# ak110/object_detector

Measured on AMD Instinct MI355X. Metric: images_per_sec, higher is better.
Workload: dtype f16

## Files before the change

object_detector_amd/csrc/conv_8ph.hip:

```cpp
#include "conv_8ph_tile.h"
#include "conv_common.h"

namespace {

struct E8Entry {
  int BM;
  bool (*variant)(int ksize, bool pw, int epi, int epi2, const void** fn, const char** name);
};
const E8Entry g_e8[] = {{256, od_conv_8ph_variant_mf4}, {224, od_conv_8ph_variant_mf3}, {192, od_conv_8ph_variant_mf2},
                        {160, od_conv_8ph_variant_mf1}};
constexpr int kNumE8 = sizeof(g_e8) / sizeof(g_e8[0]);

}

int od_conv_8ph_num_cfgs() { return kNumE8; }

long od_conv_8ph_tiles(int idx, int M, int Cout) { return (long)od_ceil_div(M, g_e8[idx].BM) * od_ceil_div(Cout, E_BN); }
double od_conv_8ph_tile_cost(int idx, int nk) { return 13.0 + 1.78 * nk * (0.5 + 0.0625 * (g_e8[idx].BM / 32)); }

bool od_conv_8ph_can_fuse_pointwise(const ConvKP& p) { return p.splitk == 1 && p.Cout == E_BN && p.Cout2 == 128; }

bool od_conv_8ph_select(int idx, const ConvKP& p, int ksize, ConvKernelInfo* info) {
  if (idx < 0 || idx >= kNumE8) return false;
  if ((p.Cin & 63) != 0 || p.tconv) return false;
  if (p.x_bytes >= 0x7F000000u || p.w_bytes >= 0x7F000000u || p.x_bytes == 0) return false;
  const E8Entry& e = g_e8[idx];
  const bool pw = p.w2 != nullptr;
  if (p.nseg > 1 && (ksize != 3 || pw || p.stride != 1 || p.res_mode != OD_RES_NONE)) return false;
  const size_t epi = (size_t)(e.BM / 2) * (E_BN + 4) * 4;
  const int epi1 = od_epi_of(p);
  const int epi2 = (pw && epi1 != OD_EPI_RT) ? od_epi(p.act2, OD_RES_NONE, false) : OD_EPI_RT;
  const void* fn;
  const char* name;
  if (!e.variant(ksize, pw, epi1, epi2, &fn, &name) &&
      !e.variant(ksize, pw, OD_EPI_RT, OD_EPI_RT, &fn, &name))
    return false;
  *info = {fn, name, e.BM, E_BN, E_BK, 512, epi > (size_t)2 * E_BUF ? epi : (size_t)2 * E_BUF};
  return true;
}
```

object_detector_amd/csrc/conv_8ph_inst.hip:

```cpp
#include "conv_8ph_kernel.h"

#ifndef OD_E8_MF1
#error "compile with -DOD_E8_MF1=1..4"
#endif

namespace {

struct E8Variant {
  int ksize;
  bool pw;
  int epi, epi2;
  const void* fn;
  const char* name;
};
#define OD_E8V(KS, PW, SEG, EPI, EPI2)                                                                                  \
  {KS, PW, EPI, EPI2, (const void*)&od_conv_8ph<KS, OD_E8_MF1, EPI, EPI2, PW, SEG>,                                     \
   "od_conv_8ph<" #KS ", " OD_STR(OD_E8_MF1) ", " OD_STR(EPI) ", " OD_STR(EPI2) ", " #PW ", " #SEG ">"}
const E8Variant g_variants[] = {
    OD_E8V(1, false, false, OD_EPI_RT, OD_EPI_RT),
    OD_E8V(1, false, false, OD_EPI_LEAKY_NONE_F16, OD_EPI_RT),
    OD_E8V(1, false, false, OD_EPI_ELU_NONE_F16, OD_EPI_RT),
    OD_E8V(1, false, false, OD_EPI_ELU_UP2_F16, OD_EPI_RT),
    OD_E8V(1, false, false, OD_EPI_ELU_NONE_F32, OD_EPI_RT),
    OD_E8V(3, false, true, OD_EPI_RT, OD_EPI_RT),
    OD_E8V(3, false, true, OD_EPI_LEAKY_NONE_F16, OD_EPI_RT),
    OD_E8V(3, false, true, OD_EPI_LEAKY_SAME_F16, OD_EPI_RT),
    OD_E8V(3, false, true, OD_EPI_ELU_NONE_F16, OD_EPI_RT),
    OD_E8V(3, false, true, OD_EPI_ELU_UP2_F16, OD_EPI_RT),
    OD_E8V(3, false, true, OD_EPI_LINEAR_NONE_F32, OD_EPI_RT),
    OD_E8V(3, false, true, OD_EPI_LEAKY_NONE_F32, OD_EPI_RT),
    OD_E8V(3, false, true, OD_EPI_ELU_NONE_F32, OD_EPI_RT),
    OD_E8V(1, true, false, OD_EPI_RT, OD_EPI_RT),
    OD_E8V(3, true, false, OD_EPI_RT, OD_EPI_RT),
    OD_E8V(3, true, false, OD_EPI_LEAKY_NONE_F16, OD_EPI_LEAKY_NONE_F16),
    OD_E8V(3, true, false, OD_EPI_LEAKY_SAME_F16, OD_EPI_LEAKY_NONE_F16),
};

}

#define OD_CAT_(a, b) a##b
#define OD_CAT(a, b) OD_CAT_(a, b)
bool OD_CAT(od_conv_8ph_variant_mf, OD_E8_MF1)(int ksize, bool pw, int epi, int epi2, const void** fn, const char** name) {
  for (const E8Variant& v : g_variants)
    if (v.ksize == ksize && v.pw == pw && v.epi == epi && v.epi2 == epi2) {
      *fn = v.fn;
      *name = v.name;
      return true;
    }
  return false;
}
```

object_detector_amd/csrc/conv_8ph_kernel.h:

```cpp
#pragma once
#include "conv_8ph_tile.h"
#include "conv_common.h"

namespace {

constexpr int E_ALO = 0, E_AHI = E_REGION, E_BLO = 2 * E_REGION, E_BHI = 3 * E_REGION;

struct TapWalk {
  int c0, tap, tapoff, dx;
  int sel_tap;
};

constexpr unsigned E_OOB = 0x80000000u;

template <int MT, int NF = 4, bool KEEP = false>
static __device__ __forceinline__ void e8_epilogue_rt(const ConvKP& p, f32x4 (&acc)[MT][NF], int m0w, int n0w, int l15,
                                                          int lq, f16x8 (*keep)[NF / 2] = nullptr, int mrows = MT * 16,
                                                          const float* pre_sc = nullptr, const float* pre_bi = nullptr) {
  unsigned pb[MT], ppix[MT];
#pragma unroll
  for (int i = 0; i < MT; ++i) {
    const int m = m0w + i * 16 + l15;
    pb[i] = (unsigned)m / (unsigned)p.HoWo;
    ppix[i] = (unsigned)m - pb[i] * (unsigned)p.HoWo;
  }
#pragma unroll
  for (int pr = 0; pr < NF / 2; ++pr) {
    const int n = n0w + (2 * pr + (lq & 1)) * 16 + (lq >> 1) * 8;
    const bool nok = n < p.Cout;
    float sc[8], bi[8];
    if (pre_sc) {
#pragma unroll
      for (int e = 0; e < 8; ++e) {
        sc[e] = pre_sc[e];
        bi[e] = pre_bi[e];
      }
    } else {
      const f32x4 s0 = *(const f32x4*)(p.scale + n), s1 = *(const f32x4*)(p.scale + n + 4);
      const f32x4 b0 = *(const f32x4*)(p.bias + n), b1 = *(const f32x4*)(p.bias + n + 4);
#pragma unroll
      for (int e = 0; e < 4; ++e) {
        sc[e] = s0[e];
        sc[4 + e] = s1[e];
        bi[e] = b0[e];
        bi[4 + e] = b1[e];
      }
    }
    f16x8 rv[MT];
#pragma unroll
    for (int i = 0; i < MT; ++i) {
      const int m = m0w + i * 16 + l15;
      f16x8 r = {0, 0, 0, 0, 0, 0, 0, 0};
      if (nok && m < p.M && p.res_mode != OD_RES_NONE) {
        long long roff;
        if (p.res_mode == OD_RES_SAME) {
          roff = (long long)m * p.Cout + n;
        } else {
          const unsigned ho = ppix[i] / (unsigned)p.Wo, wo = ppix[i] - ho * (unsigned)p.Wo;
          roff = ((long long)(pb[i] * (unsigned)(p.Ho >> 1) + (ho >> 1)) * (p.Wo >> 1) + (wo >> 1)) * p.Cout + n;
        }
        r = *(const f16x8*)(p.res + roff);
      }
      rv[i] = r;
    }
#pragma unroll
    for (int i = 0; i < MT; ++i) {
      const int m = m0w + i * 16 + l15;
      const bool ok = nok && m < p.M && i * 16 + l15 < mrows;
      float v[8];
#pragma unroll
      for (int e = 0; e < 4; ++e) {
        float a = acc[i][2 * pr][e], bq = acc[i][2 * pr + 1][e];
        od_permlane16_swap(a, bq);
        v[e] = a;
        v[4 + e] = bq;
      }
#pragma unroll
      for (int e = 0; e < 8; ++e) v[e] = v[e] * sc[e] + bi[e];
      if (p.act == OD_ACT_LEAKY) {
#pragma unroll
        for (int e = 0; e < 8; ++e) v[e] = od_leaky(v[e], p.alpha);
      } else if (p.act == OD_ACT_ELU) {
#pragma unroll
        for (int e = 0; e < 8; ++e) v[e] = v[e] > 0.f ? v[e] : p.alpha * od_expm1_fast(v[e]);
      }
      if (p.res_mode != OD_RES_NONE) {
#pragma unroll
        for (int e = 0; e < 8; ++e) v[e] += (float)rv[i][e];
      }
      if (ok) {
        const long long ooff = (long long)pb[i] * p.obs + (long long)ppix[i] * p.ops + n;
        if (p.out_f32) {
          float* o = (float*)p.out + ooff;
          *(f32x4*)o = f32x4{v[0], v[1], v[2], v[3]};
          *(f32x4*)(o + 4) = f32x4{v[4], v[5], v[6], v[7]};
        } else {
          f16x8 h;
#pragma unroll
          for (int e = 0; e < 8; ++e) h[e] = (f16)v[e];
          *(f16x8*)((f16*)p.out + ooff) = h;
        }
      }
      if (KEEP) {
        f16x8 h;
#pragma unroll
        for (int e = 0; e < 8; ++e) h[e] = (f16)v[e];
        keep[i][pr] = h;
      }
    }
  }
}

template <int EPI, int MT, int NF, bool KEEP>
static __device__ __forceinline__ void e8_epilogue_fixed(const ConvKP& p, f32x4 (&acc)[MT][NF], int m0w, int n0w, int l15, int lq,
                                                         f16x8 (*keep)[NF / 2], int mrows, const float* pre_sc,
                                                         const float* pre_bi) {
  constexpr int ACT = od_epi_act(EPI), RES = od_epi_res(EPI);
  constexpr bool F32 = od_epi_f32(EPI);
  unsigned orow[MT], rrow[RES != OD_RES_NONE ? MT : 1];
#pragma unroll
  for (int i = 0; i < MT; ++i) {
    const unsigned m = (unsigned)min(m0w + i * 16 + l15, p.M - 1);
    const unsigned b = m / (unsigned)p.HoWo, pix = m - b * (unsigned)p.HoWo;
    orow[i] = b * (unsigned)p.obs + pix * (unsigned)p.ops;
    if (RES == OD_RES_SAME) rrow[i] = m * (unsigned)p.Cout;
    if (RES == OD_RES_UP2) {
      const unsigned ho = pix / (unsigned)p.Wo, wo = pix - ho * (unsigned)p.Wo;
      rrow[i] = ((b * (unsigned)(p.Ho >> 1) + (ho >> 1)) * (unsigned)(p.Wo >> 1) + (wo >> 1)) * (unsigned)p.Cout;
    }
  }
#pragma unroll
  for (int pr = 0; pr < NF / 2; ++pr) {
    const int n = n0w + (2 * pr + (lq & 1)) * 16 + (lq >> 1) * 8;
    const bool nok = n < p.Cout;
    float sc[8], bi[8];
    if (pre_sc) {
#pragma unroll
      for (int e = 0; e < 8; ++e) {
        sc[e] = pre_sc[e];
        bi[e] = pre_bi[e];
      }
    } else {
      const f32x4 s0 = *(const f32x4*)(p.scale + n), s1 = *(const f32x4*)(p.scale + n + 4);
      const f32x4 b0 = *(const f32x4*)(p.bias + n), b1 = *(const f32x4*)(p.bias + n + 4);
#pragma unroll
      for (int e = 0; e < 4; ++e) {
        sc[e] = s0[e];
        sc[4 + e] = s1[e];
        bi[e] = b0[e];
        bi[4 + e] = b1[e];
      }
    }
    f16x8 rv[RES != OD_RES_NONE ? MT : 1];
    if (RES != OD_RES_NONE) {
      const unsigned nr = nok ? (unsigned)n : 0u;
#pragma unroll
      for (int i = 0; i < MT; ++i) rv[i] = *(const f16x8*)(p.res + (rrow[i] + nr));
    }
#pragma unroll
    for (int i = 0; i < MT; ++i) {
      f32x4 a = acc[i][2 * pr], bq = acc[i][2 * pr + 1];
      od_permlane16_swap4(a, bq);
      float v[8] = {a[0], a[1], a[2], a[3], bq[0], bq[1], bq[2], bq[3]};
#pragma unroll
      for (int e = 0; e < 8; ++e) v[e] = v[e] * sc[e] + bi[e];
      if (ACT == OD_ACT_LEAKY) {
#pragma unroll
        for (int e = 0; e < 8; ++e) v[e] = od_leaky(v[e], p.alpha);
      } else if (ACT == OD_ACT_ELU) {
#pragma unroll
        for (int e = 0; e < 8; ++e) v[e] = od_elu_select(v[e], p.alpha);
      }
      if (RES != OD_RES_NONE) {
#pragma unroll
        for (int e = 0; e < 8; ++e) v[e] += (float)rv[i][e];
      }
      f16x8 h;
      if (!F32 || KEEP) {
#pragma unroll
        for (int e = 0; e < 8; ++e) h[e] = (f16)v[e];
      }
      if (nok && m0w + i * 16 + l15 < p.M && i * 16 + l15 < mrows) {
        const unsigned ooff = orow[i] + (unsigned)n;
        if (F32) {
          float* o = (float*)p.out + ooff;
          *(f32x4*)o = f32x4{v[0], v[1], v[2], v[3]};
          *(f32x4*)(o + 4) = f32x4{v[4], v[5], v[6], v[7]};
        } else {
          *(f16x8*)((f16*)p.out + ooff) = h;
        }
      }
      if (KEEP) keep[i][pr] = h;
    }
  }
}

template <int MT, int NF = 4, bool KEEP = false, int EPI = OD_EPI_RT>
static __device__ __forceinline__ void e8_epilogue_direct(const ConvKP& p, f32x4 (&acc)[MT][NF], int m0w, int n0w, int l15,
                                                          int lq, f16x8 (*keep)[NF / 2] = nullptr, int mrows = MT * 16,
                                                          const float* pre_sc = nullptr, const float* pre_bi = nullptr) {
  if constexpr (EPI == OD_EPI_RT)
    e8_epilogue_rt<MT, NF, KEEP>(p, acc, m0w, n0w, l15, lq, keep, mrows, pre_sc, pre_bi);
  else
    e8_epilogue_fixed<EPI, MT, NF, KEEP>(p, acc, m0w, n0w, l15, lq, keep, mrows, pre_sc, pre_bi);
}

template <int KS, int MF1, int EPI, int EPI2, bool PW, bool SEG>
__global__ __launch_bounds__(512, 2) void od_conv_8ph(ConvKP p_in) {
  constexpr int MF0 = 4, MT = MF0 + MF1, WROWS = MT * 16, BM = 2 * WROWS;
  extern __shared__ __attribute__((aligned(16))) char smem[];
  const int tid = threadIdx.x;
  const int lane = tid & 63;
  const int wave = __builtin_amdgcn_readfirstlane(tid >> 6);
  const int wr = wave >> 2, wc = wave & 3;
  const int l15 = lane & 15, lq = lane >> 4;

  int logical;
  {
    const int nt = p_in.mtiles * p_in.ntiles;
    const int pid = p_in.splitk > 1 ? (int)blockIdx.x / p_in.splitk : (int)blockIdx.x;
    const int q = nt >> 3, r = nt & 7, xcd = pid & 7, loc = pid >> 3;
    logical = (xcd < r ? xcd * (q + 1) : r * (q + 1) + (xcd - r) * q) + loc;
  }
  int tm = logical / p_in.ntiles;
  const int tn = logical - tm * p_in.ntiles;
  ConvKP p_seg;
  if (SEG) p_seg = p_in;
  if (SEG && p_in.nseg > 1) {
    int sg = 0;
    if (tm >= p_in.seg_tile0[1]) sg = 1;
    if (p_in.nseg > 2 && tm >= p_in.seg_tile0[2]) sg = 2;
    tm -= p_in.seg_tile0[sg];
    p_seg.x = p_in.seg_x[sg];
    p_seg.out = p_in.seg_out[sg];
    p_seg.H = p_seg.Ho = p_in.seg_H[sg];
    p_seg.W = p_seg.Wo = p_in.seg_W[sg];
    p_seg.HoWo = p_seg.H * p_seg.W;
    p_seg.M = p_in.seg_M[sg];
    p_seg.x_bytes = (unsigned)p_seg.M * (unsigned)p_in.Cin * 2u;
    if (p_in.obs == 0) p_seg.obs = (long long)p_seg.HoWo * p_in.Cout;
  }
  const ConvKP& p = SEG ? p_seg : p_in;
  const int m0 = tm * BM, n0 = tn * E_BN;
  const int nk_all = p.Ktot / E_BK;
  const int ks0 = p.splitk > 1 ? ((int)blockIdx.x % p.splitk) * p.steps_per_split : 0;
  const int nk = p.splitk > 1 ? min(p.steps_per_split, nk_all - ks0) : nk_all;
  if (nk <= 0) return;

  const int rr = tid >> 3;
  const int lc = (tid & 7) ^ (rr & 7);
  int a_base[2][2];
  unsigned a_vmask[2][2];
  unsigned a_sel[2][2];
#pragma unroll
  for (int s = 0; s < 2; ++s)
#pragma unroll
    for (int j = 0; j < 2; ++j) {
      const int m = m0 + j * WROWS + s * 64 + rr;
      a_vmask[s][j] = 0u;
      a_base[s][j] = 0;
      if (m < p.M && (s == 0 || rr < MF1 * 16)) {
        const unsigned b = (unsigned)m / (unsigned)p.HoWo;
        const unsigned pix = (unsigned)m - b * (unsigned)p.HoWo;
        const unsigned ho = pix / (unsigned)p.Wo;
        const unsigned wo = pix - ho * (unsigned)p.Wo;
        const int hi0 = (int)ho * p.stride - p.pad, wi0 = (int)wo * p.stride - p.pad;
        a_base[s][j] = ((((int)b * p.H + hi0 + p.pad) * p.W + wi0 + p.pad) * p.Cin + lc * 8) * 2;
#pragma unroll
        for (int t = 0; t < KS * KS; ++t) {
          const int hi = hi0 + t / KS, wi = wi0 + t % KS;
          if ((unsigned)hi < (unsigned)p.H && (unsigned)wi < (unsigned)p.W) a_vmask[s][j] |= 1u << t;
        }
      }
    }
  int w_off[2][2];
#pragma unroll
  for (int s = 0; s < 2; ++s)
#pragma unroll
    for (int j = 0; j < 2; ++j) {
      const int n = n0 + (2 * j + (rr >> 5)) * 64 + s * 32 + (rr & 31);
      w_off[s][j] = (n * p.Kstride + lc * 8 + ks0 * E_BK) * 2;
    }
  const __amdgpu_buffer_rsrc_t rs_x = __builtin_amdgcn_make_buffer_rsrc(
      (void*)(p.x - (long long)p.pad * (p.W + 1) * p.Cin), 0, (int)(p.x_bytes + (unsigned)(p.pad * (p.W + 1) * p.Cin * 2)),
      0x00020000);
  const __amdgpu_buffer_rsrc_t rs_w = __builtin_amdgcn_make_buffer_rsrc((void*)p.w, 0, (int)p.w_bytes, 0x00020000);
  auto blds16 = [&](const __amdgpu_buffer_rsrc_t& rs, unsigned voff, int soff, char* lptr) {
    __builtin_amdgcn_raw_ptr_buffer_load_lds(rs, (__attribute__((address_space(3))) void*)lptr, 16, (int)voff, soff, 0, 0);
  };

  auto walk_init = [&](TapWalk& w, int kt) {
    const int k0 = kt * E_BK;
    if (KS == 3) {
      w.sel_tap = -1;
      w.tap = k0 / p.Cin;
      w.c0 = k0 - w.tap * p.Cin;
      const int dy = w.tap / 3;
      w.dx = w.tap - dy * 3;
      w.tapoff = (dy * p.W + w.dx) * p.Cin;
    } else {
      w.sel_tap = -1;
      w.tap = 0;
      w.c0 = k0;
      w.dx = 0;
      w.tapoff = 0;
    }
  };
  auto walk_next = [&](TapWalk& w) {
    w.c0 += E_BK;
    if (KS == 3 && w.c0 >= p.Cin) {
      w.c0 = 0;
      ++w.tap;
      if (++w.dx == 3) {
        w.dx = 0;
        w.tapoff += (p.W - 2) * p.Cin;
      } else {
        w.tapoff += p.Cin;
      }
    }
  };
  TapWalk walk_lo, walk_hi;
  walk_init(walk_lo, ks0);
  walk_init(walk_hi, ks0);

  char* const piece = smem + wave * 1024;
  auto stage_a = [&](int s, TapWalk& w, int buf) {
    const int koff = w.tapoff + w.c0;
    char* dst = piece + buf * E_BUF + (s ? E_AHI : E_ALO);
    if (w.sel_tap != w.tap) {
      w.sel_tap = w.tap;
#pragma unroll
      for (int j = 0; j < 2; ++j) a_sel[s][j] = ((a_vmask[s][j] >> w.tap) & 1u) ? (unsigned)a_base[s][j] : E_OOB;
    }
#pragma unroll
    for (int j = 0; j < 2; ++j) blds16(rs_x, a_sel[s][j], koff * 2, dst + j * 8192);
    walk_next(w);
  };
  auto stage_b = [&](int s, int t, int buf) {
    char* dst = piece + buf * E_BUF + (s ? E_BHI : E_BLO);
#pragma unroll
    for (int j = 0; j < 2; ++j) blds16(rs_w, (unsigned)w_off[s][j], t * (E_BK * 2), dst + j * 8192);
  };

  const int w2buf = ((nk - 1) & 1) ^ 1;
  const __amdgpu_buffer_rsrc_t rs_w2 =
      __builtin_amdgcn_make_buffer_rsrc((void*)(PW ? p.w2 : p.w), 0, (int)(PW ? p.w2_bytes : p.w_bytes), 0x00020000);
  auto stage_w2 = [&](int ks) {
#pragma unroll
    for (int h = 0; h < 2; ++h)
      blds16(rs_w2, (unsigned)(((h * 64 + rr) * p.K2stride + lc * 8) * 2), ks * (E_BK * 2),
             piece + w2buf * E_BUF + ks * E_REGION + h * 8192);
  };

  f32x4 acc[MT][4];
#pragma unroll
  for (int i = 0; i < MT; ++i)
#pragma unroll
    for (int j = 0; j < 4; ++j) acc[i][j] = f32x4{0.f, 0.f, 0.f, 0.f};

  stage_a(0, walk_lo, 0);
  stage_b(0, 0, 0);
  stage_b(1, 0, 0);
  stage_a(1, walk_hi, 0);
  if (nk > 1) {
    stage_a(0, walk_lo, 1);
    stage_b(0, 1, 1);
    wait_vmcnt<8>();
  } else {
    wait_vmcnt<0>();
  }
  __builtin_amdgcn_s_barrier();

  const int fa = (wr * 64 + l15) * 128 + ((lq ^ (l15 & 7)) * 16);
  const int fb = (wc * 32 + l15) * 128 + ((lq ^ (l15 & 7)) * 16);

  f16x8 xa[MF0][2], wlo[2][2], whi[2][2];
  auto ldf = [&](f16x8& dst, const char* src) { dst = *(const f16x8*)src; };
  auto mma = [&](f32x4& c, const f16x8& a, const f16x8& b) {
    c = __builtin_amdgcn_mfma_f32_16x16x32_f16(a, b, c, 0, 0, 0);
  };

  auto L0 = [&](int t) {
    const char* cur = smem + (t & 1) * E_BUF;
#pragma unroll
    for (int f = 0; f < 2; ++f)
#pragma unroll
      for (int kh = 0; kh < 2; ++kh) ldf(wlo[f][kh], cur + E_BLO + ((fb + f * 2048) ^ (kh * 64)));
#pragma unroll
    for (int f = 0; f < MF0; ++f)
#pragma unroll
      for (int kh = 0; kh < 2; ++kh) ldf(xa[f][kh], cur + E_ALO + ((fa + f * 2048) ^ (kh * 64)));
    if (t + 1 < nk) {
      stage_b(1, t + 1, (t & 1) ^ 1);
      wait_vmcnt<8>();
    } else if (PW) {
      stage_w2(0);
      wait_vmcnt<2>();
    } else {
      wait_vmcnt<0>();
    }
  };
  auto L1 = [&](int t) {
    const char* cur = smem + (t & 1) * E_BUF;
#pragma unroll
    for (int f = 0; f < 2; ++f)
#pragma unroll
      for (int kh = 0; kh < 2; ++kh) ldf(whi[f][kh], cur + E_BHI + ((fb + f * 2048) ^ (kh * 64)));
    if (t + 1 < nk) {
      stage_a(1, walk_hi, (t & 1) ^ 1);
      wait_vmcnt<8>();
    } else if (PW) {
      stage_w2(1);
    } else {
      wait_vmcnt<0>();
    }
  };
  auto L2 = [&](int t) {
    const char* cur = smem + (t & 1) * E_BUF;
#pragma unroll
    for (int f = 0; f < MF1; ++f)
#pragma unroll
      for (int kh = 0; kh < 2; ++kh) ldf(xa[f][kh], cur + E_AHI + ((fa + f * 2048) ^ (kh * 64)));
    if (t + 2 < nk) stage_a(0, walk_lo, t & 1);
    if (PW && t + 1 == nk) stage_w2(2);
  };
  auto L3 = [&](int t) {
    if (t + 2 < nk) {
      stage_b(0, t + 2, t & 1);
      wait_vmcnt<8>();
    } else if (PW && t + 1 == nk) {
      stage_w2(3);
    } else {
      wait_vmcnt<0>();
    }
  };
  auto M = [&](int ph) {
    __builtin_amdgcn_s_setprio(1);
#pragma unroll
    for (int kh = 0; kh < 2; ++kh)
#pragma unroll
      for (int i = 0; i < ((ph < 2) ? MF0 : MF1); ++i)
#pragma unroll
        for (int j = 0; j < 2; ++j) {
          if (ph == 0) mma(acc[i][j], wlo[j][kh], xa[i][kh]);
          if (ph == 1) mma(acc[i][2 + j], whi[j][kh], xa[i][kh]);
          if (ph == 2) mma(acc[MF0 + i][2 + j], whi[j][kh], xa[i][kh]);
          if (ph == 3) mma(acc[MF0 + i][j], wlo[j][kh], xa[i][kh]);
        }
    __builtin_amdgcn_s_setprio(0);
  };

  if (wr == 0) {
    for (int t = 0; t < nk; ++t) {
      L0(t);
      M(0);
      __builtin_amdgcn_s_barrier();
      L1(t);
      M(1);
      __builtin_amdgcn_s_barrier();
      L2(t);
      M(2);
      __builtin_amdgcn_s_barrier();
      L3(t);
      M(3);
      __builtin_amdgcn_s_barrier();
    }
  } else {
    L0(0);
    __builtin_amdgcn_s_barrier();
    for (int t = 0; t < nk; ++t) {
      M(0);
      L1(t);
      __builtin_amdgcn_s_barrier();
      M(1);
      L2(t);
      __builtin_amdgcn_s_barrier();
      M(2);
      L3(t);
      __builtin_amdgcn_s_barrier();
      M(3);
      if (t + 1 < nk) {
        L0(t + 1);
        __builtin_amdgcn_s_barrier();
      }
    }
  }
  __syncthreads();

  if constexpr (PW) {
    const int rg = wave >> 2, cg = wave & 3;
    float sc2[8], bi2[8];
    {
      const int n2 = cg * 32 + (lq & 1) * 16 + (lq >> 1) * 8;
      const f32x4 s0 = *(const f32x4*)(p.scale2 + n2), s1 = *(const f32x4*)(p.scale2 + n2 + 4);
      const f32x4 b0 = *(const f32x4*)(p.bias2 + n2), b1 = *(const f32x4*)(p.bias2 + n2 + 4);
#pragma unroll
      for (int e = 0; e < 4; ++e) {
        sc2[e] = s0[e];
        sc2[4 + e] = s1[e];
        bi2[e] = b0[e];
        bi2[4 + e] = b1[e];
      }
    }
    f16x8 ykeep[MT][2];
    od_mfma_results_ready();
    e8_epilogue_direct<MT, 4, true, EPI>(p, acc, m0 + wr * WROWS, n0 + wc * 64, l15, lq, ykeep);
    ConvKP p2 = p;
    p2.scale = p.scale2;
    p2.bias = p.bias2;
    p2.act = p.act2;
    p2.alpha = p.alpha2;
    p2.res_mode = OD_RES_NONE;
    p2.out = (void*)p.out2;
    p2.out_f32 = 0;
    p2.Cout = p.Cout2;
    p2.obs = (long long)p.HoWo * p.Cout2;
    p2.ops = p.Cout2;
    char* const ybuf = smem + (w2buf ^ 1) * E_BUF;
    const char* const wbuf = smem + w2buf * E_BUF;
    const int fy = (rg * 64 + l15) * 128 + ((lq ^ (l15 & 7)) * 16);
    const int fw = (cg * 32 + l15) * 128 + ((lq ^ (l15 & 7)) * 16);
#pragma unroll
    for (int half = 0; half < 2; ++half) {
      if (wr == half) {
#pragma unroll
        for (int i = 0; i < MT; ++i)
#pragma unroll
          for (int pr = 0; pr < 2; ++pr) {
            const int row = i * 16 + l15;
            const int chunk = (2 * pr + (lq & 1)) * 2 + (lq >> 1);
            *(f16x8*)(ybuf + wc * E_REGION + row * 128 + ((chunk ^ (row & 7)) * 16)) = ykeep[i][pr];
          }
      }
      asm volatile("s_waitcnt lgkmcnt(0)" ::: "memory");
      __builtin_amdgcn_s_barrier();
      f32x4 acc2[4][2];
#pragma unroll
      for (int i = 0; i < 4; ++i)
#pragma unroll
        for (int f = 0; f < 2; ++f) acc2[i][f] = f32x4{0.f, 0.f, 0.f, 0.f};
#pragma unroll
      for (int ks = 0; ks < 4; ++ks)
#pragma unroll
        for (int kh = 0; kh < 2; ++kh) {
          f16x8 wf[2], yf[4];
#pragma unroll
          for (int f = 0; f < 2; ++f) wf[f] = *(const f16x8*)(wbuf + ks * E_REGION + ((fw + f * 2048) ^ (kh * 64)));
#pragma unroll
          for (int i = 0; i < 4; ++i) yf[i] = *(const f16x8*)(ybuf + ks * E_REGION + ((fy + i * 2048) ^ (kh * 64)));
#pragma unroll
          for (int i = 0; i < 4; ++i)
#pragma unroll
            for (int f = 0; f < 2; ++f) acc2[i][f] = __builtin_amdgcn_mfma_f32_16x16x32_f16(wf[f], yf[i], acc2[i][f], 0, 0, 0);
        }
      od_mfma_results_ready();
      e8_epilogue_direct<4, 2, false, EPI2>(p2, acc2, m0 + half * WROWS + rg * 64, cg * 32, l15, lq, nullptr, WROWS - rg * 64, sc2, bi2);
      if (half == 0) {
        asm volatile("s_waitcnt lgkmcnt(0)" ::: "memory");
        __builtin_amdgcn_s_barrier();
      }
    }
  } else if (EPI == OD_EPI_RT && p.splitk > 1) {
    conv_epilogue<E_BN, 2, 4, MT, 4, 512>(p, smem, acc, m0, n0, tid, wr, wc, l15, lq);
  } else {
    od_mfma_results_ready();
    e8_epilogue_direct<MT, 4, false, EPI>(p, acc, m0 + wr * WROWS, n0 + wc * 64, l15, lq);
  }
}

}
```

object_detector_amd/csrc/conv_common.h:

```cpp
#pragma once
#include "common.h"

struct ConvKP {
  const f16* x;
  const f16* w;
  const float* scale;
  const float* bias;
  const f16* res;
  void* out;
  const f16* zero;
  int H, W, Cin, Ho, Wo, Cout;
  int stride, pad;
  int Kstride, Ktot, M, HoWo;
  int act;
  float alpha;
  int res_mode, out_f32;
  long long obs, ops;
  int mtiles, ntiles;
  int splitk, steps_per_split;
  float* ws;
  int Mq;
  int tconv, Hs, Ws;
  unsigned x_bytes, w_bytes;
  float* stats;
  const f16* w2;
  const float* scale2;
  const float* bias2;
  f16* out2;
  int Cout2, act2;
  float alpha2;
  unsigned w2_bytes;
  int K2stride;
  int nseg;
  int seg_tile0[4];
  const f16* seg_x[3];
  void* seg_out[3];
  int seg_H[3], seg_W[3], seg_M[3];
  int off32;
};

static __device__ __forceinline__ void glds16(const void* gptr, void* lptr) {
  __builtin_amdgcn_global_load_lds((const __attribute__((address_space(1))) void*)gptr,
                                   (__attribute__((address_space(3))) void*)lptr, 16, 0, 0);
}

static __device__ __forceinline__ float od_expm1_fast(float v) {
  const float poly = v * (1.f + v * (0.5f + v * (1.f / 6 + v * (1.f / 24 + v * (1.f / 120 + v * (1.f / 720))))));
  return v > -0.25f ? poly : __expf(v) - 1.f;
}

static __device__ __forceinline__ float od_elu_select(float v, float alpha) {
  const float poly = v * (1.f + v * (0.5f + v * (1.f / 6 + v * (1.f / 24 + v * (1.f / 120 + v * (1.f / 720))))));
  const float ex = __expf(v) - 1.f;
  const float em = v > -0.25f ? poly : ex;
  const float neg = alpha * em;
  return v > 0.f ? v : neg;
}

#define OD_EPI_RT -1
#define OD_EPI_LEAKY_NONE_F16 1
#define OD_EPI_LEAKY_SAME_F16 5
#define OD_EPI_ELU_NONE_F16 2
#define OD_EPI_ELU_UP2_F16 10
#define OD_EPI_LINEAR_NONE_F32 16
#define OD_EPI_LEAKY_NONE_F32 17
#define OD_EPI_ELU_NONE_F32 18
constexpr int od_epi(int act, int res_mode, bool out_f32) { return act | (res_mode << 2) | ((int)out_f32 << 4); }
static_assert(od_epi(OD_ACT_LEAKY, OD_RES_NONE, false) == OD_EPI_LEAKY_NONE_F16 &&
                  od_epi(OD_ACT_LEAKY, OD_RES_SAME, false) == OD_EPI_LEAKY_SAME_F16 &&
                  od_epi(OD_ACT_ELU, OD_RES_NONE, false) == OD_EPI_ELU_NONE_F16 &&
                  od_epi(OD_ACT_ELU, OD_RES_UP2, false) == OD_EPI_ELU_UP2_F16 &&
                  od_epi(OD_ACT_LINEAR, OD_RES_NONE, true) == OD_EPI_LINEAR_NONE_F32 &&
                  od_epi(OD_ACT_LEAKY, OD_RES_NONE, true) == OD_EPI_LEAKY_NONE_F32 &&
                  od_epi(OD_ACT_ELU, OD_RES_NONE, true) == OD_EPI_ELU_NONE_F32,
              "OD_EPI_* literals");
constexpr int od_epi_act(int epi) { return epi & 3; }
constexpr int od_epi_res(int epi) { return (epi >> 2) & 3; }
constexpr bool od_epi_f32(int epi) { return ((epi >> 4) & 1) != 0; }
static inline int od_epi_of(const ConvKP& p) {
  return (p.off32 && p.splitk <= 1 && !p.tconv && !p.stats) ? od_epi(p.act, p.res_mode, p.out_f32 != 0) : OD_EPI_RT;
}
#define OD_STR_(x) #x
#define OD_STR(x) OD_STR_(x)

static __device__ __forceinline__ void od_permlane16_swap(float& a, float& b) {
  asm volatile("s_nop 1\n\tv_permlane16_swap_b32 %0, %1\n\ts_nop 1" : "+v"(a), "+v"(b));
}
static __device__ __forceinline__ void od_permlane16_swap4(f32x4& a, f32x4& b) {
  float a0 = a[0], a1 = a[1], a2 = a[2], a3 = a[3], b0 = b[0], b1 = b[1], b2 = b[2], b3 = b[3];
  asm volatile(
      "s_nop 1\n\tv_permlane16_swap_b32 %0, %4\n\tv_permlane16_swap_b32 %1, %5\n\tv_permlane16_swap_b32 %2, %6\n\t"
      "v_permlane16_swap_b32 %3, %7\n\ts_nop 1"
      : "+v"(a0), "+v"(a1), "+v"(a2), "+v"(a3), "+v"(b0), "+v"(b1), "+v"(b2), "+v"(b3));
  a = f32x4{a0, a1, a2, a3};
  b = f32x4{b0, b1, b2, b3};
}
static __device__ __forceinline__ void od_mfma_results_ready() {
  __builtin_amdgcn_sched_barrier(0);
  asm volatile("s_nop 15\n\ts_nop 15" ::: "memory");
  __builtin_amdgcn_sched_barrier(0);
}

static __device__ __forceinline__ float od_leaky(float v, float alpha) { return fmaxf(v, v * alpha); }

template <int N>
static __device__ __forceinline__ void wait_vmcnt() {
  asm volatile("s_waitcnt vmcnt(%0)" ::"n"(N) : "memory");
}


static __device__ __forceinline__ int od_tconv_pixel(const ConvKP& p, unsigned m, unsigned BM) {
  const unsigned t = m / BM, r = m - t * BM;
  const unsigned cls = t & 3u, idx = (t >> 2) * BM + r;
  if (idx >= (unsigned)p.Mq) return -1;
  const unsigned HsWs = (unsigned)(p.Hs * p.Ws);
  const unsigned b = idx / HsWs, q = idx - b * HsWs;
  const unsigned i = q / (unsigned)p.Ws, j = q - i * (unsigned)p.Ws;
  return (int)(b * (unsigned)p.HoWo + (2u * i + (cls >> 1)) * (unsigned)p.Wo + 2u * j + (cls & 1u));
}

template <int BN, int WM, int WN, int MT, int NTL, int NT = WM * WN * 64, bool STATS = false, int EPI = OD_EPI_RT>
static __device__ __forceinline__ void conv_epilogue(const ConvKP& p, char* smem, f32x4 (&acc)[MT][NTL], int m0, int n0,
                                                     int tid, int wm, int wn, int l15, int lq) {
  constexpr int WTM = MT * 16, WTN = NTL * 16, SLD = BN + 4;
  constexpr bool FX = EPI != OD_EPI_RT;
  static_assert(!(FX && STATS), "the statistics epilogue has no policy");
  const int act = FX ? od_epi_act(EPI) : p.act, res_mode = FX ? od_epi_res(EPI) : p.res_mode;
  const bool out_f32 = FX ? od_epi_f32(EPI) : p.out_f32 != 0;
  const bool splitk = !FX && p.splitk > 1, tconv = !FX && p.tconv;
  float* stg = (float*)smem;
  constexpr int CH = BN / 8;
  constexpr int RPP = NT / CH;
  const int c8 = (tid % CH) * 8;
  const int n = n0 + c8;
  float sc[8], bi[8];
  if (!STATS) {
    const f32x4 s0 = *(const f32x4*)(p.scale + n), s1 = *(const f32x4*)(p.scale + n + 4);
    const f32x4 b0 = *(const f32x4*)(p.bias + n), b1 = *(const f32x4*)(p.bias + n + 4);
#pragma unroll
    for (int e = 0; e < 4; ++e) {
      sc[e] = s0[e];
      sc[4 + e] = s1[e];
      bi[e] = b0[e];
      bi[4 + e] = b1[e];
    }
  }
  float st0[STATS ? 8 : 1], st1[STATS ? 8 : 1];
  if (STATS) {
#pragma unroll
    for (int e = 0; e < 8; ++e) st0[e] = st1[e] = 0.f;
  }
  constexpr int NPASS = (WTM + RPP - 1) / RPP;
  constexpr bool RAGGED = (WTM % RPP) != 0;
  f16x8 resv[WM][NPASS];
  if (res_mode != OD_RES_NONE && !splitk) {
#pragma unroll
    for (int wr = 0; wr < WM; ++wr)
#pragma unroll
      for (int ps = 0; ps < NPASS; ++ps) {
        int m = m0 + wr * WTM + ps * RPP + tid / CH;
        f16x8 r = {0, 0, 0, 0, 0, 0, 0, 0};
        if (RAGGED && ps * RPP + tid / CH >= WTM) m = p.M;
        if (tconv && m < p.M) m = od_tconv_pixel(p, (unsigned)m, WM * MT * 16);
        if (m >= 0 && m < p.M && n < p.Cout) {
          long long roff;
          if (res_mode == OD_RES_SAME) {
            roff = (long long)m * p.Cout + n;
          } else {
            const unsigned b = (unsigned)m / (unsigned)p.HoWo;
            const unsigned pix = (unsigned)m - b * (unsigned)p.HoWo;
            const unsigned ho = pix / (unsigned)p.Wo, wo = pix - ho * (unsigned)p.Wo;
            roff = ((long long)(b * (unsigned)(p.Ho >> 1) + (ho >> 1)) * (p.Wo >> 1) + (wo >> 1)) * p.Cout + n;
          }
          r = *(const f16x8*)(p.res + roff);
        }
        resv[wr][ps] = r;
      }
  }
#pragma unroll
  for (int wr = 0; wr < WM; ++wr) {
    if (wm == wr) {
#pragma unroll
      for (int j = 0; j < NTL; ++j) {
        const int nl = wn * WTN + j * 16 + lq * 4;
#pragma unroll
        for (int i = 0; i < MT; ++i) *(f32x4*)(stg + (i * 16 + l15) * SLD + nl) = acc[i][j];
      }
    }
    __syncthreads();
    if (splitk) {
      float* slab = p.ws + (long long)((int)blockIdx.x % p.splitk) * p.M * p.Cout;
#pragma unroll
      for (int ps = 0; ps < NPASS; ++ps) {
        const int row = ps * RPP + tid / CH;
        const int m = (RAGGED && row >= WTM) ? p.M : m0 + wr * WTM + row;
        if (m < p.M && n < p.Cout) {
          float* o = slab + (long long)m * p.Cout + n;
          *(f32x4*)o = *(const f32x4*)(stg + row * SLD + c8);
          *(f32x4*)(o + 4) = *(const f32x4*)(stg + row * SLD + c8 + 4);
        }
      }
      if (wr + 1 < WM) __syncthreads();
      continue;
    }
#pragma unroll
    for (int ps = 0; ps < NPASS; ++ps) {
      const int row = ps * RPP + tid / CH;
      int m = (RAGGED && row >= WTM) ? p.M : m0 + wr * WTM + row;
      if (tconv && m < p.M) m = od_tconv_pixel(p, (unsigned)m, WM * MT * 16);
      if (m >= 0 && m < p.M && n < p.Cout) {
        const f32x4 v0 = *(const f32x4*)(stg + row * SLD + c8);
        const f32x4 v1 = *(const f32x4*)(stg + row * SLD + c8 + 4);
        float v[8] = {v0[0], v0[1], v0[2], v0[3], v1[0], v1[1], v1[2], v1[3]};
        if (!STATS) {
#pragma unroll
          for (int e = 0; e < 8; ++e) v[e] = v[e] * sc[e] + bi[e];
        }
        if (STATS) {
        } else if (act == OD_ACT_LEAKY) {
#pragma unroll
          for (int e = 0; e < 8; ++e) v[e] = od_leaky(v[e], p.alpha);
        } else if (act == OD_ACT_ELU) {
#pragma unroll
          for (int e = 0; e < 8; ++e) v[e] = FX ? od_elu_select(v[e], p.alpha) : (v[e] > 0.f ? v[e] : p.alpha * od_expm1_fast(v[e]));
        }
        if (!STATS && res_mode != OD_RES_NONE) {
#pragma unroll
          for (int e = 0; e < 8; ++e) v[e] += (float)resv[wr][ps][e];
        }
        const unsigned b = (unsigned)m / (unsigned)p.HoWo;
        const unsigned pix = (unsigned)m - b * (unsigned)p.HoWo;
        const long long ooff = FX ? (long long)(b * (unsigned)p.obs + pix * (unsigned)p.ops + (unsigned)n)
                                  : (long long)b * p.obs + (long long)pix * p.ops + n;
        if (out_f32) {
          float* o = (float*)p.out + ooff;
          *(f32x4*)o = f32x4{v[0], v[1], v[2], v[3]};
          *(f32x4*)(o + 4) = f32x4{v[4], v[5], v[6], v[7]};
        } else {
          f16x8 h;
#pragma unroll
          for (int e = 0; e < 8; ++e) h[e] = (f16)v[e];
          *(f16x8*)((f16*)p.out + ooff) = h;
          if (STATS) {
#pragma unroll
            for (int e = 0; e < 8; ++e) {
              const float q = (float)h[e];
              st0[e] += q;
              st1[e] += q * q;
            }
          }
        }
      }
    }
    if (wr + 1 < WM) __syncthreads();
  }
  if (STATS) {
    static_assert(CH == 8 || CH == 16 || CH == 32, "BN must be 64, 128 or 256");
#pragma unroll
    for (int off = CH; off < 64; off <<= 1) {
#pragma unroll
      for (int e = 0; e < 8; ++e) {
        st0[e] += __shfl_xor(st0[e], off, 64);
        st1[e] += __shfl_xor(st1[e], off, 64);
      }
    }
    __syncthreads();
    float* red = (float*)smem;
    const int wv = tid >> 6, ln = tid & 63;
    if (ln < CH) {
#pragma unroll
      for (int e = 0; e < 8; ++e) {
        red[(wv * CH + ln) * 16 + e] = st0[e];
        red[(wv * CH + ln) * 16 + 8 + e] = st1[e];
      }
    }
    __syncthreads();
    if (tid < CH && n < p.Cout) {
      float a[8], b[8];
#pragma unroll
      for (int e = 0; e < 8; ++e) a[e] = b[e] = 0.f;
      for (int w2 = 0; w2 < NT / 64; ++w2) {
#pragma unroll
        for (int e = 0; e < 8; ++e) {
          a[e] += red[(w2 * CH + tid) * 16 + e];
          b[e] += red[(w2 * CH + tid) * 16 + 8 + e];
        }
      }
      float* row = p.stats + (long long)(m0 / (WM * WTM)) * 2 * p.Cout;
#pragma unroll
      for (int e = 0; e < 8; ++e) {
        row[n + e] = a[e];
        row[p.Cout + n + e] = b[e];
      }
    }
  }
}

struct ConvKernelInfo {
  const void* fn;
  const char* name;
  int BM, BN, BK, threads;
  size_t lds;
};

int od_conv_igemm_num_cfgs();
bool od_conv_igemm_select(int cfg, int ksize, int Cin, bool want_stats, int epi, ConvKernelInfo* info);
int od_conv_finish_prepare(const ConvKP& p, od_launches* L);
int od_conv_8ph_num_cfgs();
long od_conv_8ph_tiles(int idx, int M, int Cout);
double od_conv_8ph_tile_cost(int idx, int nk);
bool od_conv_8ph_can_fuse_pointwise(const ConvKP& p);
bool od_conv_8ph_select(int idx, const ConvKP& p, int ksize, ConvKernelInfo* info);
bool od_conv_8ph_variant_mf4(int ksize, bool pw, int epi, int epi2, const void** fn, const char** name);
bool od_conv_8ph_variant_mf3(int ksize, bool pw, int epi, int epi2, const void** fn, const char** name);
bool od_conv_8ph_variant_mf2(int ksize, bool pw, int epi, int epi2, const void** fn, const char** name);
bool od_conv_8ph_variant_mf1(int ksize, bool pw, int epi, int epi2, const void** fn, const char** name);
bool od_tconv_small_supported(const od_conv_desc* d);
int od_tconv_small_prepare(od_ctx* ctx, const od_conv_desc* d, od_launches* L);
bool od_conv_rdirect_supported(const od_conv_desc* d);
int od_conv_rdirect_prepare(od_ctx* ctx, const od_conv_desc* d, od_launches* L);
bool od_conv_stream3_supported(const od_conv_desc* d);
int od_conv_stream3_prepare(od_ctx* ctx, const od_conv_desc* d, od_launches* L);
```

object_detector_amd/csrc/conv_dispatch.hip:

```cpp
#include <string.h>

#include "conv_common.h"

namespace {

int pick_cfg(const od_ctx* ctx, int M, int Cin, int Cout, int ksize, bool e8_ok, bool throughput) {
  const int cus = ctx->num_cu;
  const int cfg_e8 = od_conv_igemm_num_cfgs();
  const bool spec_ok = (Cin % 64) == 0;
  if (Cout <= 64) return (ksize == 3 && od_ceil_div(M, 128) >= 8 * cus) ? 1 : 3;
  const long t128 = (long)od_ceil_div(M, 128) * od_ceil_div(Cout, 128);
  if (ksize == 1) {
    if (!spec_ok) return 3;
    if (M <= 4096) return (M >= 2048 && Cin >= 512) ? 6 : 3;
    if (M <= 16384) return 7;
    if (Cout < 256) return 3;
    if (t128 < cus) return 4;
  }
  if (!spec_ok) return t128 >= 2L * cus ? 0 : 2;
  const int nk = od_ceil_div(ksize * ksize * Cin, 64);
  if (throughput && e8_ok && ksize == 3 && Cout >= 192 && M >= 2048) {
    double best = t128 >= cus ? t128 * (7.5 + 1.07 * nk) * 0.5 : t128 * (10.0 + 0.55 * nk);
    int pick = t128 >= cus ? 4 : (Cout <= 256 ? 7 : 5);
    for (int i = 0; i < od_conv_8ph_num_cfgs(); ++i) {
      const long tiles = od_conv_8ph_tiles(i, M, Cout);
      if (tiles * 3 < cus) continue;
      const double c = (double)tiles * od_conv_8ph_tile_cost(i, nk);
      if (c < 0.95 * best) {
        best = c / 0.95;
        pick = cfg_e8 + i;
      }
    }
    return pick;
  }
  if (t128 >= cus) {
    if (Cout == 128) return 2;
    const double c13 = (double)od_ceil_div((int)t128, 2 * cus) * (7.5 + 1.07 * nk);
    double best = 0.93 * c13;
    int pick = 4;
    for (int i = 0; e8_ok && i < od_conv_8ph_num_cfgs(); ++i) {
      const double c = (double)((od_conv_8ph_tiles(i, M, Cout) + cus - 1) / cus) * od_conv_8ph_tile_cost(i, nk);
      if (c < best) {
        best = c;
        pick = cfg_e8 + i;
      }
    }
    return pick;
  }
  if (Cout <= 256) return M < 2048 ? 3 : 7;
  return (M >= 2048 && 2 * t128 <= cus) ? 7 : 5;
}

int conv_describe(const od_ctx* ctx, const od_conv_desc* d, bool want_stats, od_conv_desc* v, ConvKP* kp) {
  if (d && d->nseg > 1) {
    OD_REQUIRE(d->nseg <= 3, "od_conv2d_fwd: nseg %d > 3", d->nseg);
    OD_REQUIRE(d->ksize == 3 && d->stride == 1 && d->res_mode == OD_RES_NONE && !d->w2 && !want_stats && !d->transposed,
               "od_conv2d_fwd: a grouped launch (nseg > 1) is a 3x3 stride-1 layer without residual / w2 / bn_partials / "
               "transposed mode");
    for (int i = 0; i < d->nseg; ++i)
      OD_REQUIRE(d->seg_x[i] && d->seg_out[i] && d->seg_H[i] > 0 && d->seg_W[i] > 0, "od_conv2d_fwd: segment %d is incomplete", i);
  }
  OD_REQUIRE(ctx && d, "od_conv2d_fwd: null ctx/desc");
  *v = *d;
  const bool grouped = d->nseg > 1;
  if (grouped) {
    v->x = d->seg_x[0];
    v->out = d->seg_out[0];
    v->H = d->seg_H[0];
    v->W = d->seg_W[0];
  }
  d = v;
  OD_REQUIRE(d->x && d->w && d->scale && d->bias && d->out, "od_conv2d_fwd: null tensor");
  OD_REQUIRE(d->ksize == 1 || d->ksize == 3, "od_conv2d_fwd: ksize %d unsupported", d->ksize);
  OD_REQUIRE(d->stride == 1 || d->stride == 2, "od_conv2d_fwd: stride %d unsupported", d->stride);
  OD_REQUIRE(d->B > 0 && d->H > 0 && d->W > 0 && d->Cin > 0 && d->Cout > 0, "od_conv2d_fwd: bad dims");
  OD_REQUIRE(d->Cin % 8 == 0 && d->Cout % 8 == 0, "od_conv2d_fwd: Cin/Cout must be multiples of 8 (got %d/%d)",
             d->Cin, d->Cout);
  OD_REQUIRE(d->res_mode == OD_RES_NONE || d->res, "od_conv2d_fwd: res_mode set but res is null");
  OD_REQUIRE(d->act >= OD_ACT_LINEAR && d->act <= OD_ACT_ELU, "od_conv2d_fwd: bad act");
  OD_REQUIRE(d->act != OD_ACT_LEAKY || (d->alpha >= 0.f && d->alpha <= 1.f), "od_conv2d_fwd: leaky slope must be in [0, 1]");
  ConvKP& p = *kp;
  p.pad = d->ksize / 2;
  p.tconv = d->transposed != 0;
  if (p.tconv)
    OD_REQUIRE(d->ksize == 3 && d->stride == 2 && d->Cin % 64 == 0,
               "od_conv2d_fwd: transposed mode is the backward-data of a 3x3 stride-2 conv (Cin %% 64 == 0)");
  p.H = p.tconv ? 2 * d->H : d->H;
  p.W = p.tconv ? 2 * d->W : d->W;
  p.stride = p.tconv ? 1 : d->stride;
  p.Hs = d->H;
  p.Ws = d->W;
  p.Ho = (p.H + 2 * p.pad - d->ksize) / p.stride + 1;
  p.Wo = (p.W + 2 * p.pad - d->ksize) / p.stride + 1;
  if (d->res_mode == OD_RES_UP2)
    OD_REQUIRE(p.Ho % 2 == 0 && p.Wo % 2 == 0, "od_conv2d_fwd: OD_RES_UP2 needs even output size");
  const long long M64 = (long long)d->B * p.Ho * p.Wo;
  OD_REQUIRE(M64 * d->Cout < (1LL << 31) && (long long)d->B * d->H * d->W * d->Cin < (1LL << 31),
             "od_conv2d_fwd: tensor too large for 32-bit element offsets");
  p.HoWo = p.Ho * p.Wo;
  long long Mg = 0;
  long long seg_x_max = 0;
  for (int i = 0; grouped && i < d->nseg; ++i) {
    const long long Mi = (long long)d->B * d->seg_H[i] * d->seg_W[i];
    Mg += Mi;
    seg_x_max = seg_x_max > Mi * d->Cin ? seg_x_max : Mi * d->Cin;
  }
  OD_REQUIRE(!grouped || (Mg * d->Cout < (1LL << 31) && seg_x_max < (1LL << 31)),
             "od_conv2d_fwd: grouped launch too large for 32-bit element offsets");
  p.M = grouped ? (int)Mg : (int)M64;
  p.nseg = grouped ? d->nseg : 0;

  if (want_stats)
    OD_REQUIRE(!p.tconv && d->out_dtype == OD_DT_F16 && d->act == OD_ACT_LINEAR && d->res_mode == OD_RES_NONE,
               "od_conv2d_fwd: bn_partials needs the raw convolution (f16 output, no activation, no residual, no transposed "
               "gather; scale / bias are NOT applied)");
  if (d->w2) {
    OD_REQUIRE(d->scale2 && d->bias2 && d->out2 && d->Cout2 > 0 && d->Cout2 % 8 == 0,
               "od_conv2d_fwd: w2 needs scale2, bias2, out2 and Cout2 (a multiple of 8)");
    OD_REQUIRE(d->act2 >= OD_ACT_LINEAR && d->act2 <= OD_ACT_ELU, "od_conv2d_fwd: bad act2");
    OD_REQUIRE(d->act2 != OD_ACT_LEAKY || (d->alpha2 >= 0.f && d->alpha2 <= 1.f), "od_conv2d_fwd: leaky slope (alpha2) must be in [0, 1]");
    OD_REQUIRE(d->out_dtype == OD_DT_F16 && !p.tconv && !want_stats && d->Cout % 8 == 0 &&
                   (d->out_batch_stride == 0 || d->out_batch_stride == (long long)p.HoWo * d->Cout) &&
                   (d->out_pix_stride == 0 || d->out_pix_stride == d->Cout),
               "od_conv2d_fwd: w2 (the consuming pointwise layer) needs a dense f16 output of the first layer");
  }
  p.x = (const f16*)d->x;
  p.w = (const f16*)d->w;
  p.scale = d->scale;
  p.bias = d->bias;
  p.res = (const f16*)d->res;
  p.out = d->out;
  p.zero = (const f16*)ctx->zero_page;
  p.Cin = d->Cin;
  p.Cout = d->Cout;
  p.Ktot = d->ksize * d->ksize * d->Cin;
  p.Kstride = od_round_up(p.Ktot, 64);
  p.act = d->act;
  p.alpha = d->alpha;
  p.res_mode = d->res_mode;
  p.out_f32 = d->out_dtype == OD_DT_F32;
  p.stats = d->bn_partials;
  p.w2 = nullptr;
  p.scale2 = d->scale2;
  p.bias2 = d->bias2;
  p.out2 = (f16*)d->out2;
  p.Cout2 = d->Cout2;
  p.act2 = d->act2;
  p.alpha2 = d->alpha2;
  p.K2stride = od_round_up(d->Cout, 64);
  p.w2_bytes = (unsigned)((long long)od_round_up(d->Cout2 > 0 ? d->Cout2 : 1, 256) * p.K2stride * 2);
  p.x_bytes = (unsigned)((grouped ? seg_x_max : (long long)d->B * d->H * d->W * d->Cin) * 2);
  p.w_bytes = (unsigned)((long long)od_round_up(d->Cout, 256) * p.Kstride * 2);
  p.obs = d->out_batch_stride ? d->out_batch_stride : (long long)p.HoWo * d->Cout;
  p.ops = d->out_pix_stride ? d->out_pix_stride : d->Cout;
  long long hw_max = p.HoWo;
  for (int i = 0; grouped && i < d->nseg; ++i) hw_max = hw_max > (long long)d->seg_H[i] * d->seg_W[i] ? hw_max : (long long)d->seg_H[i] * d->seg_W[i];
  p.off32 = p.obs >= 0 && p.ops >= 0 && (long long)d->B * p.obs < (1LL << 31) &&
            (long long)(d->B - 1) * p.obs + (hw_max - 1) * p.ops + d->Cout < (1LL << 31);
  p.splitk = 1;
  p.steps_per_split = 0;
  p.ws = (float*)d->splitk_workspace;
  return OD_OK;
}

int conv_choose_cfg(const od_ctx* ctx, const od_conv_desc* d, const ConvKP& p, bool want_stats, int* cfg_out) {
  int cfg = d->tile_cfg;
  if (cfg < 0)
    cfg = pick_cfg(ctx, p.M, d->Cin, d->Cout, d->ksize, !want_stats && !p.tconv && (long long)p.x_bytes < 0x7F000000LL, cfg == -2);
  const int cfg_e8 = od_conv_igemm_num_cfgs();
  OD_REQUIRE(cfg < cfg_e8 + od_conv_8ph_num_cfgs(), "od_conv2d_fwd: tile_cfg %d out of range", cfg);
  OD_REQUIRE(!(want_stats && cfg >= cfg_e8), "od_conv2d_fwd: bn_partials is supported by the table kernels only (tile_cfg %d)", cfg);
  OD_REQUIRE(!p.tconv || cfg < cfg_e8, "od_conv2d_fwd: transposed mode runs on the table kernels only (tile_cfg %d)", cfg);
  *cfg_out = cfg;
  return OD_OK;
}

int conv_select(int cfg, const od_conv_desc* d, const ConvKP& p, bool want_stats, ConvKernelInfo* k) {
  const int cfg_e8 = od_conv_igemm_num_cfgs();
  if (cfg >= cfg_e8) {
    if (od_conv_8ph_select(cfg - cfg_e8, p, d->ksize, k)) return OD_OK;
    od_set_error("od_conv2d_fwd: tile_cfg %d (8-phase kernel) needs Cin %% 64 == 0 and no transposed gather", cfg);
    return OD_ERR_INVALID;
  }
  if (od_conv_igemm_select(cfg, d->ksize, d->Cin, want_stats, od_epi_of(p), k)) return OD_OK;
  od_set_error("od_conv2d_fwd: tile_cfg %d needs Cin %% %d == 0 for 3x3 (Cin = %d); use cfg 0-3", cfg, k->BK, d->Cin);
  return OD_ERR_INVALID;
}

void conv_tile_kp(const od_conv_desc* d, const ConvKernelInfo& k, ConvKP* kp) {
  ConvKP& p = *kp;
  p.mtiles = od_ceil_div(p.M, k.BM);
  if (p.nseg > 1) {
    int t0 = 0;
    for (int i = 0; i < 3; ++i) {
      const bool used = i < d->nseg;
      p.seg_tile0[i] = t0;
      p.seg_x[i] = used ? (const f16*)d->seg_x[i] : nullptr;
      p.seg_out[i] = used ? d->seg_out[i] : nullptr;
      p.seg_H[i] = used ? d->seg_H[i] : 0;
      p.seg_W[i] = used ? d->seg_W[i] : 0;
      p.seg_M[i] = d->B * p.seg_H[i] * p.seg_W[i];
      t0 += od_ceil_div(p.seg_M[i], k.BM);
    }
    p.seg_tile0[3] = t0;
    p.mtiles = t0;
    if (!d->out_batch_stride) p.obs = 0;
  }
  p.Mq = 0;
  if (p.tconv) {
    p.Mq = p.M / 4;
    p.mtiles = 4 * od_ceil_div(p.Mq, k.BM);
    p.M = p.mtiles * k.BM;
  }
  p.ntiles = od_ceil_div(d->Cout, k.BN);
}

int conv_prepare(od_ctx* ctx, const od_conv_desc* desc, bool want_stats, od_launches* L) {
  od_conv_desc v;
  ConvKP p;
  if (int rc = conv_describe(ctx, desc, want_stats, &v, &p)) return rc;
  const od_conv_desc* d = &v;
  const bool grouped = p.nseg > 1;
  if (d->tile_cfg < 0 && !want_stats && !grouped) {
    if (p.tconv && od_tconv_small_supported(d)) return od_tconv_small_prepare(ctx, d, L);
    if (od_conv_rdirect_supported(d)) return od_conv_rdirect_prepare(ctx, d, L);
    if (!p.tconv && od_conv_stream3_supported(d)) return od_conv_stream3_prepare(ctx, d, L);
  }
  int cfg;
  if (int rc = conv_choose_cfg(ctx, d, p, want_stats, &cfg)) return rc;
  const bool use_e8 = cfg >= od_conv_igemm_num_cfgs();
  if (grouped && !(use_e8 && d->Cin % 64 == 0)) {
    od_conv_desc q = *d;
    q.nseg = 0;
    for (int i = 0; i < d->nseg; ++i) {
      q.x = d->seg_x[i];
      q.out = d->seg_out[i];
      q.H = d->seg_H[i];
      q.W = d->seg_W[i];
      if (int rc = conv_prepare(ctx, &q, false, L)) return rc;
    }
    return OD_OK;
  }
  ConvKernelInfo k;
  if (int rc = conv_select(cfg, d, p, want_stats, &k)) return rc;
  conv_tile_kp(d, k, &p);
  if (d->bn_partials) {
    const long long need = (long long)p.mtiles * 2 * d->Cout * 4;
    if (d->bn_partials_bytes < need) {
      od_set_error("od_conv2d_fwd: bn_partials holds %lld bytes, %d rows x 2 x %d channels need %lld", (long long)d->bn_partials_bytes,
                   p.mtiles, d->Cout, need);
      return OD_ERR_WORKSPACE;
    }
  }
  if (d->splitk_workspace && d->splitk != 1 && !p.tconv && !want_stats && !grouped) {
    const int cus = ctx->num_cu;
    const int tiles = p.mtiles * p.ntiles;
    const int nk = od_ceil_div(p.Ktot, k.BK);
    constexpr int thr_mul = 8;
    constexpr int tgt_mul = 1;
    int sk = d->splitk > 1 ? d->splitk : ((tiles * thr_mul <= cus && nk >= 8) ? od_ceil_div(tgt_mul * cus / 2, tiles) : 1);
    if (sk > nk / 4) sk = nk / 4;
    const long long slab_bytes = (long long)p.M * d->Cout * 4;
    if ((long long)sk * slab_bytes > (long long)d->splitk_workspace_bytes) sk = (int)(d->splitk_workspace_bytes / slab_bytes);
    if (sk > 1) {
      p.steps_per_split = od_ceil_div(nk, sk);
      p.splitk = od_ceil_div(nk, p.steps_per_split);
    }
  }
  if (d->w2 && use_e8 && od_conv_8ph_can_fuse_pointwise(p)) p.w2 = (const f16*)d->w2;
  if (int rc = conv_select(cfg, d, p, want_stats, &k)) return rc;
  if (int rc = od_ensure_lds(ctx, k.fn, k.lds)) return rc;
  const size_t launch_lds = (use_e8 && p.splitk <= 1 && k.lds > (size_t)128 * 1024) ? (size_t)128 * 1024 : k.lds;
  if (int rc = od_add_launch(L, {k.name, od_issue_kp, k.fn, dim3(p.mtiles * p.ntiles * p.splitk), dim3(k.threads), launch_lds}, p))
    return rc;
  if (p.splitk > 1)
    if (int rc = od_conv_finish_prepare(p, L)) return rc;
  if (!d->w2 || p.w2) return OD_OK;
  od_conv_desc q;
  memset(&q, 0, sizeof(q));
  q.x = d->out;
  q.w = d->w2;
  q.scale = d->scale2;
  q.bias = d->bias2;
  q.out = d->out2;
  q.B = d->B;
  q.H = p.Ho;
  q.W = p.Wo;
  q.Cin = d->Cout;
  q.Cout = d->Cout2;
  q.ksize = 1;
  q.stride = 1;
  q.act = d->act2;
  q.alpha = d->alpha2;
  q.res_mode = OD_RES_NONE;
  q.out_dtype = OD_DT_F16;
  q.tile_cfg = d->tile_cfg < 0 ? d->tile_cfg : -1;
  q.splitk = d->splitk;
  q.splitk_workspace = d->splitk_workspace;
  q.splitk_workspace_bytes = d->splitk_workspace_bytes;
  return conv_prepare(ctx, &q, false, L);
}

}

extern "C" int od_conv_num_tile_cfgs(void) { return od_conv_igemm_num_cfgs() + od_conv_8ph_num_cfgs(); }

extern "C" int od_conv_weight_dims(int cout, int cin, int ksize, int* cout_pad, int* kpad) {
  OD_REQUIRE(cout > 0 && cin > 0 && (ksize == 1 || ksize == 3), "od_conv_weight_dims: bad dims");
  if (cout_pad) *cout_pad = od_round_up(cout, 256);
  if (kpad) *kpad = od_round_up(ksize * ksize * cin, 64);
  return OD_OK;
}

int od_conv_prepare(od_ctx* ctx, const od_conv_desc* d, od_launches* L) {
  return conv_prepare(ctx, d, d && d->bn_partials, L);
}

extern "C" int od_conv2d_fwd(od_ctx* ctx, const od_conv_desc* d, void* stream) {
  return od_prepare_issue(stream, od_conv_prepare, ctx, d);
}

extern "C" int od_conv2d_fwd_bn_rows(od_ctx* ctx, const od_conv_desc* d) {
  od_conv_desc v;
  ConvKP p;
  ConvKernelInfo k;
  int cfg;
  if (conv_describe(ctx, d, true, &v, &p) || conv_choose_cfg(ctx, &v, p, true, &cfg) || conv_select(cfg, &v, p, true, &k)) return -1;
  conv_tile_kp(&v, k, &p);
  return p.mtiles;
}

extern "C" int od_conv2d_bwd_data(od_ctx* ctx, const void* dz, const void* w_bwd, const void* dx_accumulate, void* dx, int B,
                                  int Ho, int Wo, int Cin, int Cout, int ksize, int stride, void* stream) {
  OD_REQUIRE(ctx && dz && w_bwd && dx, "od_conv2d_bwd_data: null argument");
  OD_REQUIRE(Cin > 0 && Cin <= 2048, "od_conv2d_bwd_data: Cin out of range (1..2048)");
  od_conv_desc d;
  memset(&d, 0, sizeof(d));
  d.x = dz;
  d.w = w_bwd;
  d.scale = ctx->ones;
  d.bias = (const float*)ctx->zero_page;
  d.res = dx_accumulate;
  d.res_mode = dx_accumulate ? OD_RES_SAME : OD_RES_NONE;
  d.out = dx;
  d.B = B;
  d.H = Ho;
  d.W = Wo;
  d.Cin = Cout;
  d.Cout = Cin;
  d.ksize = ksize;
  d.stride = stride;
  d.act = OD_ACT_LINEAR;
  d.out_dtype = OD_DT_F16;
  d.tile_cfg = -1;
  d.transposed = stride == 2;
  d.splitk = 1;
  return od_conv2d_fwd(ctx, &d, stream);
}
```

object_detector_amd/net.py:

```python
from __future__ import annotations

import ctypes as C
import os

import numpy as np
import torch

from . import _lib, desc, weights as W


def _stream_ptr():
    return C.c_void_p(torch.cuda.current_stream().cuda_stream)


class Context:

    _by_device = {}

    def __init__(self, device_index: int):
        self.lib = _lib.load()
        h = C.c_void_p()
        _lib.check(self.lib.od_ctx_create(device_index, C.byref(h)), "od_ctx_create")
        self.handle = h
        self.device_index = device_index

    @classmethod
    def get(cls, device) -> "Context":
        dev = torch.device(device)
        if dev.type != "cuda":
            raise _lib.OdError(f"object_detector_amd runs on MI355X only (got device {dev}); there is no CPU path")
        idx = dev.index if dev.index is not None else torch.cuda.current_device()
        if idx not in cls._by_device:
            cls._by_device[idx] = cls(idx)
        return cls._by_device[idx]


def pack_conv_weight(w_ohwi: np.ndarray):
    cout, k, _, cin = w_ohwi.shape
    cout_pad, kpad = _lib.conv_weight_dims(cout, cin, k)
    out = np.zeros((cout_pad, kpad), np.float16)
    out[:cout, :k * k * cin] = w_ohwi.reshape(cout, k * k * cin).astype(np.float16)
    return out


def pack_first_weight(w_ohwi: np.ndarray):
    cout = w_ohwi.shape[0]
    out = np.zeros((cout, 32), np.float16)
    out[:, :27] = w_ohwi.reshape(cout, 27).astype(np.float16)
    return out


def pad_vec(v: np.ndarray, n: int):
    out = np.zeros(n, np.float32)
    out[:len(v)] = v
    return out


def pack_layer(w_ohwi: np.ndarray, scale, bias, first=False):
    wp = pack_first_weight(w_ohwi) if first else pack_conv_weight(w_ohwi)
    return wp, pad_vec(np.asarray(scale, np.float32), wp.shape[0]), pad_vec(np.asarray(bias, np.float32), wp.shape[0])


MIXED_STREAM_STAGES = (4, 5)
MIXED_SPLIT = ("n.lat4", "n.lat5", "n.out3", "n.out4", "h.t0", "h.out")
_NECK_CONSUMERS = {"n.lat5": ("h.t0",), "n.lat4": ("n.out4",), "n.out4": ("h.t0",), "n.lat3": ("n.out3",), "n.out3": ("h.t0",),
                   "h.t0": ("h.out",)}


class Net:

    def __init__(self, params, batch_size, input_size=(320, 320), device="cuda:0", backbone_act=("leaky", 0.1),
                 head_act=("elu", 1.0), tile_cfg=None, overlapped=False, share_weights_with=None, precision=None,
                 stream_stages=None, split=None, wide_fpn=None):
        self.wide_fpn = True if wide_fpn is None else bool(wide_fpn)
        self.precision = precision or os.environ.get("OD_PRECISION", "f16")
        if self.precision not in ("f16", "mixed"):
            raise ValueError(f"precision must be 'f16' or 'mixed', got {self.precision!r}")
        self.stream_stages = tuple(stream_stages if stream_stages is not None else MIXED_STREAM_STAGES)
        self.split = tuple(split if split is not None else MIXED_SPLIT)
        if self.precision == "f16":
            self.stream_stages, self.split, self.wide_fpn = (), (), False
        if any(k not in (3, 4, 5) for k in self.stream_stages):
            raise ValueError("stream_stages: stages 3, 4, 5 only (stages 1-2 run as fused residual blocks)")
        for nm in self.split:
            if nm not in ("n.lat3", "n.lat4", "n.lat5", "n.out3", "n.out4", "h.t0", "h.out"):
                raise ValueError(f"split: {nm!r} is not a neck / prediction-module layer")
            if nm.startswith("n.lat") and int(nm[-1]) not in self.stream_stages:
                raise ValueError(f"split layer {nm} reads the stage-{nm[-1]} tap: that stage must be in stream_stages")
        self.ctx = Context.get(device)
        self.lib = self.ctx.lib
        self.device = torch.device(device)
        self.B = int(batch_size)
        self.H, self.W = int(input_size[0]), int(input_size[1])
        if self.H % 32 or self.W % 32:
            raise ValueError("input_size must be a multiple of 32 (three maps at stride 8/16/32)")
        self.num_classes, self.neck_ch, self.tower = W.infer_arch(params)
        self.C = 2 + self.num_classes + 4
        self.level_hw = [(self.H // s, self.W // s) for s in (8, 16, 32)]
        self.P = sum(h * w for h, w in self.level_hw) * W.NUM_PRIORS
        self.tile_cfg = dict(tile_cfg or {})
        self.auto_cfg = -2 if overlapped else -1
        self.fuse_blocks = os.environ.get("OD_FUSE_BLOCKS", "1") != "0"
        self.splitk = True
        self._splitk_elems = 0
        self._splitk_descs = []
        self._keep = []
        self._dev = {}
        if share_weights_with is not None:
            self._dev = share_weights_with._dev
        for name, cin, cout, k, _s, _bn in ([] if share_weights_with is not None else
                                            W.layer_specs(self.num_classes, self.neck_ch, self.tower)):
            w = params[name + ".w"]
            assert w.shape == (cout, k, k, cin), (name, w.shape)
            scale, bias = W.fold_bn(params, name)
            first = name == "b.conv0"
            if first:
                scale = (scale / np.float32(255.0)).astype(np.float32)
            self._dev[name] = tuple(self._to_dev(a) for a in pack_layer(w, scale, bias, first))
            if name in self.split:
                self._dev[name + "#split"] = (self._to_dev(pack_conv_weight(np.concatenate([w, w], axis=3))),) + self._dev[name][1:]
        self.input = torch.zeros((self.B, self.H, self.W, 3), dtype=torch.uint8, device=self.device)
        self.pred = torch.zeros((self.B, self.P, self.C), dtype=torch.float32, device=self.device)
        self.ops = []
        self.op_info = []
        self._hilo = {}
        self._build(backbone_act, head_act)
        if self._splitk_elems:
            nbytes = min(32 * self._splitk_elems * 4, 256 << 20)
            self.splitk_ws = torch.empty(nbytes, dtype=torch.uint8, device=self.device)
            for i in self._splitk_descs:
                desc.set_splitk(self.ops[i].conv, 0, self.splitk_ws, nbytes)
        abl = [q.partition("*") for q in filter(None, os.environ.get("OD_ABLATE_OPS", "").split(","))]
        self.ablated = bool(abl)
        if abl and os.environ.get("OD_ALLOW_ABLATION") != "1":
            raise _lib.OdError("OD_ABLATE_OPS is set (a TIMING ablation: it drops layers, results are garbage) without "
                               "OD_ALLOW_ABLATION=1; unset it")
        if abl:
            import warnings
            warnings.warn(f"OD_ABLATE_OPS={os.environ['OD_ABLATE_OPS']!r}: layers dropped from the plan, outputs are garbage")
            seen, occ = {}, []
            for inf in self.op_info:
                occ.append(f'{inf["name"]}#{seen.get(inf["name"], 0)}')
                seen[inf["name"]] = seen.get(inf["name"], 0) + 1
            keep = [i for i, inf in enumerate(self.op_info)
                    if not any((inf["name"].startswith(pre) and inf["name"].endswith(suf)) or occ[i] == pre + _s + suf
                               for pre, _s, suf in abl)]
            self.ops = [self.ops[i] for i in keep]
            self.op_info = [self.op_info[i] for i in keep]
        arr = (_lib.PlanOp * len(self.ops))(*self.ops)
        h = C.c_void_p()
        _lib.check(self.lib.od_plan_create(self.ctx.handle, arr, len(self.ops), C.byref(h)), "od_plan_create")
        self.plan = h
        self._captured = False

    def _to_dev(self, a: np.ndarray):
        t = torch.from_numpy(np.ascontiguousarray(a)).to(self.device)
        self._keep.append(t)
        return t

    def _buf(self, h, w, c):
        t = torch.empty((self.B, h, w, c), dtype=torch.float16, device=self.device)
        self._keep.append(t)
        return t

    def _buf32(self, h, w, c):
        t = torch.empty((self.B, h, w, c), dtype=torch.float32, device=self.device)
        self._keep.append(t)
        return t

    def _emit(self, kind, d, /, **info):
        self.ops.append(desc.plan_op(kind, d))
        self.op_info.append(info)

    def _wide(self, name, y32, res, res_f32, out32, out16, hilo, h, w, c, up2=False):
        m = self.B * h * w
        nbytes = m * c * (4 + (0 if res is None else (4 if res_f32 else 2)) + (4 if out32 is not None else 0)
                          + (2 if out16 is not None else 0) + (4 if hilo is not None else 0))
        self._emit(_lib.OD_OP_WIDE, desc.wide(y32, res, out32, out16, hilo, m, c, h, w, res_f32=res_f32, up2=up2),
                   name=name, flops=0.0, bytes=float(nbytes), shape=(m, c, 0), kind="wide", y=y32, res=res,
                   res_f32=bool(res_f32), out32=out32, out16=out16, hilo=hilo)

    def _neck_conv(self, name, x, x_hilo, h, w, cin, cout, k, act, up16=None, up32=None, need16=False, keep32=False,
                   consumers=None):
        consumers = _NECK_CONSUMERS.get(name, ()) if consumers is None else consumers
        want_hilo = any(c in self.split for c in consumers)
        want16 = need16 or any(c not in self.split for c in consumers)
        src, cin_eff, wkey = x, cin, None
        if name in self.split:
            if x_hilo is None:
                raise ValueError(f"split layer {name}: its input has no (hi, lo) pair")
            src, cin_eff, wkey = x_hilo, 2 * cin, name + "#split"
        if not want_hilo and up32 is None and not keep32:
            out, _, _ = self._conv(name, src, h, w, cin_eff, cout, k, 1, act, res=up16,
                                   res_mode=_lib.OD_RES_UP2 if up16 is not None else _lib.OD_RES_NONE, wkey=wkey)
            return out, None, None
        y32 = self._buf32(h, w, cout)
        in_epilogue = up16 if up32 is None else None
        self._conv(name, src, h, w, cin_eff, cout, k, 1, act, res=in_epilogue,
                   res_mode=_lib.OD_RES_UP2 if in_epilogue is not None else _lib.OD_RES_NONE, out=y32, out_f32=True, wkey=wkey)
        out16 = self._buf(h, w, cout) if want16 else None
        hilo = self._buf(h, w, 2 * cout) if want_hilo else None
        s32 = self._buf32(h, w, cout) if (keep32 and up32 is not None) else None
        if out16 is not None or hilo is not None or s32 is not None:
            self._wide(name + ".wide", y32, up32, True, s32, out16, hilo, h, w, cout, up2=up32 is not None)
        return out16, hilo, (s32 if s32 is not None else y32)

    def _conv(self, name, x, h, w, cin, cout, k, stride, act, res=None, res_mode=_lib.OD_RES_NONE, out=None,
              out_f32=False, obs=0, ops=0, then=None, wkey=None):
        ho, wo = (h + stride - 1) // stride, (w + stride - 1) // stride
        if out is None:
            out = self._buf(ho, wo, cout)
        tile_cfg = self.tile_cfg.get(name, self.auto_cfg)
        for pat, cfg in self.tile_cfg.items():
            pre, star, suf = pat.partition("*")
            if star and name.startswith(pre) and name.endswith(suf):
                tile_cfg = cfg
        out2 = None
        if then is not None:
            name2, cout2, act2 = then
            out2 = self._buf(ho, wo, cout2)
        d = desc.conv(x, *self._dev[wkey or name], out, self.B, h, w, cin, cout, k, stride, act, res=res, res_mode=res_mode,
                      out_f32=out_f32, out_batch_stride=obs, out_pix_stride=ops, tile_cfg=tile_cfg,
                      then=None if then is None else self._dev[name2] + (out2, cout2, act2))
        m = self.B * ho * wo
        if self.splitk and m * cout <= (1 << 22):
            self._splitk_elems = max(self._splitk_elems, m * cout)
            self._splitk_descs.append(len(self.ops))
        split = wkey is not None and wkey.endswith("#split")
        flops = 2.0 * m * cout * k * k * cin * (0.5 if split else 1.0)
        nbytes = float(self.B * h * w * cin * 2 + m * cout * (4 if out_f32 else 2) + cout * k * k * cin * 2
                       + (m * cout * 2 if res_mode == _lib.OD_RES_SAME else 0)
                       + (m * cout // 2 if res_mode == _lib.OD_RES_UP2 else 0))
        extra = {"split": True} if split else {}
        if then is not None:
            flops += 2.0 * m * cout2 * cout
            nbytes += float(m * cout2 * 2 + cout2 * cout * 2)
            extra["then"] = dict(name=name2, out=out2, act=act2)
        self._emit(_lib.OD_OP_CONV, d, name=name, flops=flops, bytes=nbytes, shape=(m, cout, k * k * cin),
                   kind="conv", x=x, res=res, res_mode=res_mode, out=None if isinstance(out, int) else out,
                   stride=stride, ksize=k, act=act, out_f32=out_f32, **extra)
        return (out, ho, wo) if then is None else (out, ho, wo, out2)

    def _conv_grouped(self, name, xs, dims, cin, cout, act, outs=None, out_f32=False, obs=0, ops=0):
        bufs = [self._buf(h, w, cout) for h, w in dims] if outs is None else [None] * len(dims)
        d = desc.conv_grouped(xs, dims, bufs if outs is None else outs, *self._dev[name], self.B, cin, cout, act,
                              out_f32=out_f32, out_batch_stride=obs, out_pix_stride=ops,
                              tile_cfg=self.tile_cfg.get(name, self.auto_cfg))
        m = sum(self.B * h * w for h, w in dims)
        if self.splitk and max(self.B * h * w for h, w in dims) * cout <= (1 << 22):
            self._splitk_elems = max(self._splitk_elems, max(self.B * h * w for h, w in dims) * cout)
            self._splitk_descs.append(len(self.ops))
        self._emit(_lib.OD_OP_CONV, d, name=name, flops=2.0 * m * cout * 9 * cin,
                   bytes=float(m * cin * 2 + m * cout * (4 if out_f32 else 2) + cout * 9 * cin * 2), shape=(m, cout, 9 * cin),
                   kind="conv_group", xs=list(xs), dims=list(dims), outs=bufs, act=act, out_f32=out_f32)
        return bufs

    def _bneck(self, name, x, h, w, ch, act):
        out = self._buf(h, w, ch)
        m = self.B * h * w
        d = desc.bneck(x, *self._dev[name + ".a"], *self._dev[name + ".b"], out, self.B, h, w, ch, act)
        self._emit(_lib.OD_OP_BNECK, d, name=name, flops=2.0 * m * (ch * (ch // 2) + 9 * (ch // 2) * ch),
                   bytes=float(2 * m * ch * 2 + (ch * ch // 2 + 9 * ch * ch // 2) * 2),
                   shape=(m, ch, 10 * (ch // 2)), kind="bneck", x=x, out=out, act=act)
        return out

    def _build(self, bact, hact):
        B, H, Wd = self.B, self.H, self.W
        fuse_stem = self.fuse_blocks and self.lib.od_stem_supported(H, Wd)
        if fuse_stem:
            x = self._buf(H // 2, Wd // 2, 64)
            m1 = B * (H // 2) * (Wd // 2)
            d = desc.stem(self.input, *self._dev["b.conv0"], *self._dev["b.down1"], x, B, H, Wd, bact)
            self._emit(_lib.OD_OP_STEM, d, name="b.stem", flops=2.0 * B * H * Wd * 32 * 27 + 2.0 * m1 * 64 * 288,
                       bytes=float(B * H * Wd * 3 + m1 * 64 * 2), shape=(m1, 64, 288 + 27),
                       kind="stem", x=self.input, out=x, act=bact)
        else:
            x = self._buf(H, Wd, 32)
            d = desc.conv(self.input, *self._dev["b.conv0"], x, B, H, Wd, 3, 32, 3, 1, bact, tile_cfg=0)
            self._emit(_lib.OD_OP_CONV_FIRST, d, name="b.conv0", flops=2.0 * B * H * Wd * 32 * 27,
                       bytes=float(B * H * Wd * (3 + 64)), shape=(B * H * Wd, 32, 27),
                       kind="first", x=self.input, out=x, act=bact)
        h, w, cin = H, Wd, 32
        taps = []
        for si, (n, ch) in enumerate(W.STAGES, start=1):
            fused_block = self.fuse_blocks and self.lib.od_bottleneck_supported(h // 2, w // 2, ch)
            ride = self.fuse_blocks and ch == 256 and not fused_block
            wide = si in self.stream_stages
            if wide:
                ride = False
                hilo_tap = f"n.lat{si}" in self.split
                x32 = y32 = None
            t = None
            if si == 1 and fuse_stem:
                h, w = h // 2, w // 2
            elif ride:
                x, h, w, t = self._conv(f"b.down{si}", x, h, w, cin, ch, 3, 2, bact, then=(f"b.s{si}.0.a", ch // 2, bact))
            else:
                x, h, w = self._conv(f"b.down{si}", x, h, w, cin, ch, 3, 2, bact)
            for r in range(n):
                if fused_block:
                    x = self._bneck(f"b.s{si}.{r}", x, h, w, ch, bact)
                    continue
                if t is None:
                    t, _, _ = self._conv(f"b.s{si}.{r}.a", x, h, w, ch, ch // 2, 1, 1, bact)
                if wide:
                    if y32 is None:
                        y32 = self._buf32(h, w, ch)
                        x32 = self._buf32(h, w, ch)
                    self._conv(f"b.s{si}.{r}.b", t, h, w, ch // 2, ch, 3, 1, bact, out=y32, out_f32=True)
                    last = r + 1 == n
                    xn = self._buf(h, w, ch)
                    hl = self._buf(h, w, 2 * ch) if (last and hilo_tap) else None
                    self._wide(f"b.s{si}.{r}.add", y32, x if r == 0 else x32, r != 0, x32, xn, hl, h, w, ch)
                    x = xn
                    if hl is not None:
                        self._hilo[f"tap{si}"] = hl
                    t = None
                elif ride and r + 1 < n:
                    x, _, _, t = self._conv(f"b.s{si}.{r}.b", t, h, w, ch // 2, ch, 3, 1, bact, res=x,
                                            res_mode=_lib.OD_RES_SAME, then=(f"b.s{si}.{r + 1}.a", ch // 2, bact))
                else:
                    x, _, _ = self._conv(f"b.s{si}.{r}.b", t, h, w, ch // 2, ch, 3, 1, bact, res=x,
                                         res_mode=_lib.OD_RES_SAME)
                    t = None
            cin = ch
            taps.append((x, h, w, ch))
        (c3, h3, w3, ch3), (c4, h4, w4, ch4), (c5, h5, w5, ch5) = taps[2], taps[3], taps[4]
        nc = self.neck_ch
        wf = self.precision == "mixed" and self.wide_fpn
        p5, p5s, p5w = self._neck_conv("n.lat5", c5, self._hilo.get("tap5"), h5, w5, ch5, nc, 1, hact, need16=not wf, keep32=wf)
        m4, m4s, _ = self._neck_conv("n.lat4", c4, self._hilo.get("tap4"), h4, w4, ch4, nc, 1, hact,
                                     up16=None if wf else p5, up32=p5w if wf else None)
        p4, p4s, p4w = self._neck_conv("n.out4", m4, m4s, h4, w4, nc, nc, 3, hact, need16=not wf, keep32=wf)
        m3, m3s, _ = self._neck_conv("n.lat3", c3, self._hilo.get("tap3"), h3, w3, ch3, nc, 1, hact,
                                     up16=None if wf else p4, up32=p4w if wf else None)
        p3, p3s, _ = self._neck_conv("n.out3", m3, m3s, h3, w3, nc, nc, 3, hact)
        self.levels = [(p3, h3, w3), (p4, h4, w4), (p5, h5, w5)]
        self.taps = [c3, c4, c5]
        off = 0
        cout = W.NUM_PRIORS * self.C
        group = self.precision == "f16" and self.tower == 1 and nc % 64 == 0
        if group:
            dims = [(h, w) for _x, h, w in self.levels]
            ts = self._conv_grouped("h.t0", [x for x, _h, _w in self.levels], dims, nc, nc, hact)
            ptrs, rows = [], []
            for h, w in dims:
                ptrs.append(self.pred.data_ptr() + off * self.C * 4)
                rows.append((off, h * w * W.NUM_PRIORS))
                off += h * w * W.NUM_PRIORS
            self._conv_grouped("h.out", ts, dims, nc, cout, None, outs=ptrs, out_f32=True, obs=self.P * self.C, ops=cout)
            self.op_info[-1]["pred_rows"] = rows
        for (x, h, w), xs in ([] if group else zip(self.levels, (p3s, p4s, p5s))):
            t, ts = x, xs
            for i in range(self.tower):
                t, ts, _ = self._neck_conv(f"h.t{i}", t, ts, h, w, nc, nc, 3, hact,
                                           consumers=(f"h.t{i + 1}",) if i + 1 < self.tower else ("h.out",))
            out_ptr = self.pred.data_ptr() + off * self.C * 4
            if "h.out" in self.split:
                self._conv("h.out", ts, h, w, 2 * nc, cout, 3, 1, None, out=out_ptr, out_f32=True,
                           obs=self.P * self.C, ops=cout, wkey="h.out#split")
            else:
                self._conv("h.out", t, h, w, nc, cout, 3, 1, None, out=out_ptr, out_f32=True,
                           obs=self.P * self.C, ops=cout)
            self.op_info[-1]["pred_rows"] = (off, h * w * W.NUM_PRIORS)
            off += h * w * W.NUM_PRIORS
        assert off == self.P

    def forward(self, x_u8: torch.Tensor | None = None, graph: bool = False) -> torch.Tensor:
        if x_u8 is not None:
            if x_u8.shape != self.input.shape or x_u8.dtype != torch.uint8:
                raise ValueError(f"expected uint8 {tuple(self.input.shape)}, got {x_u8.dtype} {tuple(x_u8.shape)}")
            self.input.copy_(x_u8, non_blocking=True)
        if graph:
            if not self._captured:
                s = torch.cuda.Stream(device=self.device)
                s.wait_stream(torch.cuda.current_stream())
                with torch.cuda.stream(s):
                    _lib.check(self.lib.od_plan_capture(self.plan, C.c_void_p(s.cuda_stream)), "od_plan_capture")
                torch.cuda.current_stream().wait_stream(s)
                self._captured = True
            _lib.check(self.lib.od_plan_replay(self.plan, _stream_ptr()), "od_plan_replay")
        else:
            _lib.check(self.lib.od_plan_run(self.plan, _stream_ptr()), "od_plan_run")
        return self.pred

    def time_ops(self):
        n = len(self.ops)
        ms = (C.c_float * n)()
        _lib.check(self.lib.od_plan_time_ops(self.plan, _stream_ptr(), ms, n), "od_plan_time_ops")
        names = [self.lib.od_plan_op_kernel_name(self.plan, i).decode() for i in range(n)]
        return list(ms), names

    def __del__(self):
        try:
            if getattr(self, "plan", None):
                self.lib.od_plan_destroy(self.plan)
        except Exception:
            pass
```

Baseline: 22780.

## Add sequential multi-pass conv kernel fusing trailing pointwise conv for wider outputs

Adds a sequential form of the 8-phase conv kernel in which each workgroup owns one M tile, loops over all N tiles of the first conv writing to the output, then runs a final pass computing the 1x1 pointwise conv from the freshly written output. This lets the 3x3 downsample plus following 1x1 ride together for 512-channel stages (Cout up to 1024), removing a separate launch and its dependency gap. In exchange the grid shrinks to mtiles workgroups, split-K is disabled, and the pointwise pass rereads the output through global memory, which may reduce parallelism and occupancy on small layers.

```diff
diff --git a/object_detector_amd/csrc/conv_8ph.hip b/object_detector_amd/csrc/conv_8ph.hip
--- a/object_detector_amd/csrc/conv_8ph.hip
+++ b/object_detector_amd/csrc/conv_8ph.hip
@@ -5,7 +5,7 @@
 
 struct E8Entry {
   int BM;
-  bool (*variant)(int ksize, bool pw, int epi, int epi2, const void** fn, const char** name);
+  bool (*variant)(int ksize, int pw, int epi, int epi2, const void** fn, const char** name);
 };
 const E8Entry g_e8[] = {{256, od_conv_8ph_variant_mf4}, {224, od_conv_8ph_variant_mf3}, {192, od_conv_8ph_variant_mf2},
                         {160, od_conv_8ph_variant_mf1}};
@@ -18,14 +18,21 @@
 long od_conv_8ph_tiles(int idx, int M, int Cout) { return (long)od_ceil_div(M, g_e8[idx].BM) * od_ceil_div(Cout, E_BN); }
 double od_conv_8ph_tile_cost(int idx, int nk) { return 13.0 + 1.78 * nk * (0.5 + 0.0625 * (g_e8[idx].BM / 32)); }
 
-bool od_conv_8ph_can_fuse_pointwise(const ConvKP& p) { return p.splitk == 1 && p.Cout == E_BN && p.Cout2 == 128; }
+int od_conv_8ph_can_fuse_pointwise(const ConvKP& p) {
+  if (p.splitk != 1) return 0;
+  if (p.Cout == E_BN && p.Cout2 == 128) return 1;
+  if (p.Cout % E_BK == 0 && p.Cout > E_BN && p.Cout <= 1024 && p.Cout2 <= E_BN && p.nseg <= 1 &&
+      (long long)p.M * p.Cout * 2 < 0x7F000000LL)
+    return 2;
+  return 0;
+}
 
 bool od_conv_8ph_select(int idx, const ConvKP& p, int ksize, ConvKernelInfo* info) {
   if (idx < 0 || idx >= kNumE8) return false;
   if ((p.Cin & 63) != 0 || p.tconv) return false;
   if (p.x_bytes >= 0x7F000000u || p.w_bytes >= 0x7F000000u || p.x_bytes == 0) return false;
   const E8Entry& e = g_e8[idx];
-  const bool pw = p.w2 != nullptr;
+  const int pw = p.w2 == nullptr ? 0 : (p.Cout > E_BN ? 2 : 1);
   if (p.nseg > 1 && (ksize != 3 || pw || p.stride != 1 || p.res_mode != OD_RES_NONE)) return false;
   const size_t epi = (size_t)(e.BM / 2) * (E_BN + 4) * 4;
   const int epi1 = od_epi_of(p);
diff --git a/object_detector_amd/csrc/conv_8ph_inst.hip b/object_detector_amd/csrc/conv_8ph_inst.hip
--- a/object_detector_amd/csrc/conv_8ph_inst.hip
+++ b/object_detector_amd/csrc/conv_8ph_inst.hip
@@ -8,7 +8,7 @@
 
 struct E8Variant {
   int ksize;
-  bool pw;
+  int pw;
   int epi, epi2;
   const void* fn;
   const char* name;
@@ -16,6 +16,9 @@
 #define OD_E8V(KS, PW, SEG, EPI, EPI2)                                                                                  \
   {KS, PW, EPI, EPI2, (const void*)&od_conv_8ph<KS, OD_E8_MF1, EPI, EPI2, PW, SEG>,                                     \
    "od_conv_8ph<" #KS ", " OD_STR(OD_E8_MF1) ", " OD_STR(EPI) ", " OD_STR(EPI2) ", " #PW ", " #SEG ">"}
+#define OD_E8Q(KS, EPI, EPI2)                                                                                           \
+  {KS, 2, EPI, EPI2, (const void*)&od_conv_8ph_seq<KS, OD_E8_MF1, EPI, EPI2>,                                           \
+   "od_conv_8ph_seq<" #KS ", " OD_STR(OD_E8_MF1) ", " OD_STR(EPI) ", " OD_STR(EPI2) ">"}
 const E8Variant g_variants[] = {
     OD_E8V(1, false, false, OD_EPI_RT, OD_EPI_RT),
     OD_E8V(1, false, false, OD_EPI_LEAKY_NONE_F16, OD_EPI_RT),
@@ -34,13 +37,17 @@
     OD_E8V(3, true, false, OD_EPI_RT, OD_EPI_RT),
     OD_E8V(3, true, false, OD_EPI_LEAKY_NONE_F16, OD_EPI_LEAKY_NONE_F16),
     OD_E8V(3, true, false, OD_EPI_LEAKY_SAME_F16, OD_EPI_LEAKY_NONE_F16),
+    OD_E8Q(1, OD_EPI_RT, OD_EPI_RT),
+    OD_E8Q(3, OD_EPI_RT, OD_EPI_RT),
+    OD_E8Q(3, OD_EPI_LEAKY_NONE_F16, OD_EPI_LEAKY_NONE_F16),
+    OD_E8Q(3, OD_EPI_LEAKY_SAME_F16, OD_EPI_LEAKY_NONE_F16),
 };
 
 }
 
 #define OD_CAT_(a, b) a##b
 #define OD_CAT(a, b) OD_CAT_(a, b)
-bool OD_CAT(od_conv_8ph_variant_mf, OD_E8_MF1)(int ksize, bool pw, int epi, int epi2, const void** fn, const char** name) {
+bool OD_CAT(od_conv_8ph_variant_mf, OD_E8_MF1)(int ksize, int pw, int epi, int epi2, const void** fn, const char** name) {
   for (const E8Variant& v : g_variants)
     if (v.ksize == ksize && v.pw == pw && v.epi == epi && v.epi2 == epi2) {
       *fn = v.fn;
diff --git a/object_detector_amd/csrc/conv_8ph_kernel.h b/object_detector_amd/csrc/conv_8ph_kernel.h
--- a/object_detector_amd/csrc/conv_8ph_kernel.h
+++ b/object_detector_amd/csrc/conv_8ph_kernel.h
@@ -205,8 +205,9 @@
     e8_epilogue_fixed<EPI, MT, NF, KEEP>(p, acc, m0w, n0w, l15, lq, keep, mrows, pre_sc, pre_bi);
 }
 
-template <int KS, int MF1, int EPI, int EPI2, bool PW, bool SEG>
-__global__ __launch_bounds__(512, 2) void od_conv_8ph(ConvKP p_in) {
+template <int KS, int MF1, int EPI, int EPI2, bool PW, bool SEG, bool SEQ>
+static __device__ __forceinline__ void e8_body(const ConvKP& p_in) {
+  static_assert(!(SEQ && (PW || SEG)), "the sequential form has neither the in-epilogue layer nor a segment table");
   constexpr int MF0 = 4, MT = MF0 + MF1, WROWS = MT * 16, BM = 2 * WROWS;
   extern __shared__ __attribute__((aligned(16))) char smem[];
   const int tid = threadIdx.x;
@@ -217,13 +218,13 @@
 
   int logical;
   {
-    const int nt = p_in.mtiles * p_in.ntiles;
+    const int nt = SEQ ? p_in.mtiles : p_in.mtiles * p_in.ntiles;
     const int pid = p_in.splitk > 1 ? (int)blockIdx.x / p_in.splitk : (int)blockIdx.x;
     const int q = nt >> 3, r = nt & 7, xcd = pid & 7, loc = pid >> 3;
     logical = (xcd < r ? xcd * (q + 1) : r * (q + 1) + (xcd - r) * q) + loc;
   }
-  int tm = logical / p_in.ntiles;
-  const int tn = logical - tm * p_in.ntiles;
+  int tm = SEQ ? logical : logical / p_in.ntiles;
+  const int tn = SEQ ? 0 : logical - tm * p_in.ntiles;
   ConvKP p_seg;
   if (SEG) p_seg = p_in;
   if (SEG && p_in.nseg > 1) {
@@ -241,11 +242,11 @@
     if (p_in.obs == 0) p_seg.obs = (long long)p_seg.HoWo * p_in.Cout;
   }
   const ConvKP& p = SEG ? p_seg : p_in;
-  const int m0 = tm * BM, n0 = tn * E_BN;
+  const int m0 = tm * BM;
   const int nk_all = p.Ktot / E_BK;
   const int ks0 = p.splitk > 1 ? ((int)blockIdx.x % p.splitk) * p.steps_per_split : 0;
-  const int nk = p.splitk > 1 ? min(p.steps_per_split, nk_all - ks0) : nk_all;
-  if (nk <= 0) return;
+  const int nk_conv = p.splitk > 1 ? min(p.steps_per_split, nk_all - ks0) : nk_all;
+  if (nk_conv <= 0) return;
 
   const int rr = tid >> 3;
   const int lc = (tid & 7) ^ (rr & 7);
@@ -273,299 +274,345 @@
         }
       }
     }
-  int w_off[2][2];
-#pragma unroll
-  for (int s = 0; s < 2; ++s)
-#pragma unroll
-    for (int j = 0; j < 2; ++j) {
-      const int n = n0 + (2 * j + (rr >> 5)) * 64 + s * 32 + (rr & 31);
-      w_off[s][j] = (n * p.Kstride + lc * 8 + ks0 * E_BK) * 2;
-    }
-  const __amdgpu_buffer_rsrc_t rs_x = __builtin_amdgcn_make_buffer_rsrc(
-      (void*)(p.x - (long long)p.pad * (p.W + 1) * p.Cin), 0, (int)(p.x_bytes + (unsigned)(p.pad * (p.W + 1) * p.Cin * 2)),
-      0x00020000);
-  const __amdgpu_buffer_rsrc_t rs_w = __builtin_amdgcn_make_buffer_rsrc((void*)p.w, 0, (int)p.w_bytes, 0x00020000);
   auto blds16 = [&](const __amdgpu_buffer_rsrc_t& rs, unsigned voff, int soff, char* lptr) {
     __builtin_amdgcn_raw_ptr_buffer_load_lds(rs, (__attribute__((address_space(3))) void*)lptr, 16, (int)voff, soff, 0, 0);
   };
-
-  auto walk_init = [&](TapWalk& w, int kt) {
-    const int k0 = kt * E_BK;
-    if (KS == 3) {
-      w.sel_tap = -1;
-      w.tap = k0 / p.Cin;
-      w.c0 = k0 - w.tap * p.Cin;
-      const int dy = w.tap / 3;
-      w.dx = w.tap - dy * 3;
-      w.tapoff = (dy * p.W + w.dx) * p.Cin;
-    } else {
-      w.sel_tap = -1;
-      w.tap = 0;
-      w.c0 = k0;
-      w.dx = 0;
-      w.tapoff = 0;
-    }
-  };
-  auto walk_next = [&](TapWalk& w) {
-    w.c0 += E_BK;
-    if (KS == 3 && w.c0 >= p.Cin) {
-      w.c0 = 0;
-      ++w.tap;
-      if (++w.dx == 3) {
+  f32x4 acc[MT][4];
+
+  const int npass = SEQ ? p.ntiles + 1 : 1;
+  for (int pass = 0; pass < npass; ++pass) {
+    const bool pw_pass = SEQ && pass == p.ntiles;
+    const int n0 = SEQ ? (pw_pass ? 0 : pass * E_BN) : tn * E_BN;
+    const int nk = pw_pass ? p.Cout / E_BK : nk_conv;
+    const int cin_w = pw_pass ? 0x40000000 : p.Cin;
+    if (SEQ && pw_pass) {
+      wait_vmcnt<0>();
+      __builtin_amdgcn_s_barrier();
+#pragma unroll
+      for (int s = 0; s < 2; ++s)
+#pragma unroll
+        for (int j = 0; j < 2; ++j) {
+          const int m = m0 + j * WROWS + s * 64 + rr;
+          const bool ok = m < p.M && (s == 0 || rr < MF1 * 16);
+          a_vmask[s][j] = ok ? 1u : 0u;
+          a_base[s][j] = ok ? (m * p.Cout + lc * 8) * 2 : 0;
+        }
+    }
+    int w_off[2][2];
+#pragma unroll
+    for (int s = 0; s < 2; ++s)
+#pragma unroll
+      for (int j = 0; j < 2; ++j) {
+        const int n = n0 + (2 * j + (rr >> 5)) * 64 + s * 32 + (rr & 31);
+        w_off[s][j] = (n * (pw_pass ? p.K2stride : p.Kstride) + lc * 8 + ks0 * E_BK) * 2;
+      }
+    const __amdgpu_buffer_rsrc_t rs_x = __builtin_amdgcn_make_buffer_rsrc(
+        pw_pass ? (void*)p.out : (void*)(p.x - (long long)p.pad * (p.W + 1) * p.Cin), 0,
+        pw_pass ? p.M * p.Cout * 2 : (int)(p.x_bytes + (unsigned)(p.pad * (p.W + 1) * p.Cin * 2)), 0x00020000);
+    const __amdgpu_buffer_rsrc_t rs_w = __builtin_amdgcn_make_buffer_rsrc(pw_pass ? (void*)p.w2 : (void*)p.w, 0,
+                                                                          (int)(pw_pass ? p.w2_bytes : p.w_bytes), 0x00020000);
+
+    auto walk_init = [&](TapWalk& w, int kt) {
+      const int k0 = kt * E_BK;
+      if (KS == 3) {
+        w.sel_tap = -1;
+        w.tap = k0 / cin_w;
+        w.c0 = k0 - w.tap * cin_w;
+        const int dy = w.tap / 3;
+        w.dx = w.tap - dy * 3;
+        w.tapoff = (dy * p.W + w.dx) * p.Cin;
+      } else {
+        w.sel_tap = -1;
+        w.tap = 0;
+        w.c0 = k0;
         w.dx = 0;
-        w.tapoff += (p.W - 2) * p.Cin;
-      } else {
-        w.tapoff += p.Cin;
-      }
-    }
-  };
-  TapWalk walk_lo, walk_hi;
-  walk_init(walk_lo, ks0);
-  walk_init(walk_hi, ks0);
-
-  char* const piece = smem + wave * 1024;
-  auto stage_a = [&](int s, TapWalk& w, int buf) {
-    const int koff = w.tapoff + w.c0;
-    char* dst = piece + buf * E_BUF + (s ? E_AHI : E_ALO);
-    if (w.sel_tap != w.tap) {
-      w.sel_tap = w.tap;
-#pragma unroll
-      for (int j = 0; j < 2; ++j) a_sel[s][j] = ((a_vmask[s][j] >> w.tap) & 1u) ? (unsigned)a_base[s][j] : E_OOB;
-    }
-#pragma unroll
-    for (int j = 0; j < 2; ++j) blds16(rs_x, a_sel[s][j], koff * 2, dst + j * 8192);
-    walk_next(w);
-  };
-  auto stage_b = [&](int s, int t, int buf) {
-    char* dst = piece + buf * E_BUF + (s ? E_BHI : E_BLO);
-#pragma unroll
-    for (int j = 0; j < 2; ++j) blds16(rs_w, (unsigned)w_off[s][j], t * (E_BK * 2), dst + j * 8192);
-  };
-
-  const int w2buf = ((nk - 1) & 1) ^ 1;
-  const __amdgpu_buffer_rsrc_t rs_w2 =
-      __builtin_amdgcn_make_buffer_rsrc((void*)(PW ? p.w2 : p.w), 0, (int)(PW ? p.w2_bytes : p.w_bytes), 0x00020000);
-  auto stage_w2 = [&](int ks) {
-#pragma unroll
-    for (int h = 0; h < 2; ++h)
-      blds16(rs_w2, (unsigned)(((h * 64 + rr) * p.K2stride + lc * 8) * 2), ks * (E_BK * 2),
-             piece + w2buf * E_BUF + ks * E_REGION + h * 8192);
-  };
-
-  f32x4 acc[MT][4];
-#pragma unroll
-  for (int i = 0; i < MT; ++i)
-#pragma unroll
-    for (int j = 0; j < 4; ++j) acc[i][j] = f32x4{0.f, 0.f, 0.f, 0.f};
-
-  stage_a(0, walk_lo, 0);
-  stage_b(0, 0, 0);
-  stage_b(1, 0, 0);
-  stage_a(1, walk_hi, 0);
-  if (nk > 1) {
-    stage_a(0, walk_lo, 1);
-    stage_b(0, 1, 1);
-    wait_vmcnt<8>();
-  } else {
-    wait_vmcnt<0>();
-  }
-  __builtin_amdgcn_s_barrier();
-
-  const int fa = (wr * 64 + l15) * 128 + ((lq ^ (l15 & 7)) * 16);
-  const int fb = (wc * 32 + l15) * 128 + ((lq ^ (l15 & 7)) * 16);
-
-  f16x8 xa[MF0][2], wlo[2][2], whi[2][2];
-  auto ldf = [&](f16x8& dst, const char* src) { dst = *(const f16x8*)src; };
-  auto mma = [&](f32x4& c, const f16x8& a, const f16x8& b) {
-    c = __builtin_amdgcn_mfma_f32_16x16x32_f16(a, b, c, 0, 0, 0);
-  };
-
-  auto L0 = [&](int t) {
-    const char* cur = smem + (t & 1) * E_BUF;
-#pragma unroll
-    for (int f = 0; f < 2; ++f)
-#pragma unroll
-      for (int kh = 0; kh < 2; ++kh) ldf(wlo[f][kh], cur + E_BLO + ((fb + f * 2048) ^ (kh * 64)));
-#pragma unroll
-    for (int f = 0; f < MF0; ++f)
-#pragma unroll
-      for (int kh = 0; kh < 2; ++kh) ldf(xa[f][kh], cur + E_ALO + ((fa + f * 2048) ^ (kh * 64)));
-    if (t + 1 < nk) {
-      stage_b(1, t + 1, (t & 1) ^ 1);
+        w.tapoff = 0;
+      }
+    };
+    auto walk_next = [&](TapWalk& w) {
+      w.c0 += E_BK;
+      if (KS == 3 && w.c0 >= cin_w) {
+        w.c0 = 0;
+        ++w.tap;
+        if (++w.dx == 3) {
+          w.dx = 0;
+          w.tapoff += (p.W - 2) * p.Cin;
+        } else {
+          w.tapoff += p.Cin;
+        }
+      }
+    };
+    TapWalk walk_lo, walk_hi;
+    walk_init(walk_lo, ks0);
+    walk_init(walk_hi, ks0);
+
+    char* const piece = smem + wave * 1024;
+    auto stage_a = [&](int s, TapWalk& w, int buf) {
+      const int koff = w.tapoff + w.c0;
+      char* dst = piece + buf * E_BUF + (s ? E_AHI : E_ALO);
+      if (w.sel_tap != w.tap) {
+        w.sel_tap = w.tap;
+#pragma unroll
+        for (int j = 0; j < 2; ++j) a_sel[s][j] = ((a_vmask[s][j] >> w.tap) & 1u) ? (unsigned)a_base[s][j] : E_OOB;
+      }
+#pragma unroll
+      for (int j = 0; j < 2; ++j) blds16(rs_x, a_sel[s][j], koff * 2, dst + j * 8192);
+      walk_next(w);
+    };
+    auto stage_b = [&](int s, int t, int buf) {
+      char* dst = piece + buf * E_BUF + (s ? E_BHI : E_BLO);
+#pragma unroll
+      for (int j = 0; j < 2; ++j) blds16(rs_w, (unsigned)w_off[s][j], t * (E_BK * 2), dst + j * 8192);
+    };
+
+    const int w2buf = ((nk - 1) & 1) ^ 1;
+    const __amdgpu_buffer_rsrc_t rs_w2 =
+        __builtin_amdgcn_make_buffer_rsrc((void*)(PW ? p.w2 : p.w), 0, (int)(PW ? p.w2_bytes : p.w_bytes), 0x00020000);
+    auto stage_w2 = [&](int ks) {
+#pragma unroll
+      for (int h = 0; h < 2; ++h)
+        blds16(rs_w2, (unsigned)(((h * 64 + rr) * p.K2stride + lc * 8) * 2), ks * (E_BK * 2),
+               piece + w2buf * E_BUF + ks * E_REGION + h * 8192);
+    };
+
+#pragma unroll
+    for (int i = 0; i < MT; ++i)
+#pragma unroll
+      for (int j = 0; j < 4; ++j) acc[i][j] = f32x4{0.f, 0.f, 0.f, 0.f};
+
+    stage_a(0, walk_lo, 0);
+    stage_b(0, 0, 0);
+    stage_b(1, 0, 0);
+    stage_a(1, walk_hi, 0);
+    if (nk > 1) {
+      stage_a(0, walk_lo, 1);
+      stage_b(0, 1, 1);
       wait_vmcnt<8>();
-    } else if (PW) {
-      stage_w2(0);
-      wait_vmcnt<2>();
     } else {
       wait_vmcnt<0>();
     }
-  };
-  auto L1 = [&](int t) {
-    const char* cur = smem + (t & 1) * E_BUF;
-#pragma unroll
-    for (int f = 0; f < 2; ++f)
-#pragma unroll
-      for (int kh = 0; kh < 2; ++kh) ldf(whi[f][kh], cur + E_BHI + ((fb + f * 2048) ^ (kh * 64)));
-    if (t + 1 < nk) {
-      stage_a(1, walk_hi, (t & 1) ^ 1);
-      wait_vmcnt<8>();
-    } else if (PW) {
-      stage_w2(1);
+    __builtin_amdgcn_s_barrier();
+
+    const int fa = (wr * 64 + l15) * 128 + ((lq ^ (l15 & 7)) * 16);
+    const int fb = (wc * 32 + l15) * 128 + ((lq ^ (l15 & 7)) * 16);
+
+    f16x8 xa[MF0][2], wlo[2][2], whi[2][2];
+    auto ldf = [&](f16x8& dst, const char* src) { dst = *(const f16x8*)src; };
+    auto mma = [&](f32x4& c, const f16x8& a, const f16x8& b) {
+      c = __builtin_amdgcn_mfma_f32_16x16x32_f16(a, b, c, 0, 0, 0);
+    };
+
+    auto L0 = [&](int t) {
+      const char* cur = smem + (t & 1) * E_BUF;
+#pragma unroll
+      for (int f = 0; f < 2; ++f)
+#pragma unroll
+        for (int kh = 0; kh < 2; ++kh) ldf(wlo[f][kh], cur + E_BLO + ((fb + f * 2048) ^ (kh * 64)));
+#pragma unroll
+      for (int f = 0; f < MF0; ++f)
+#pragma unroll
+        for (int kh = 0; kh < 2; ++kh) ldf(xa[f][kh], cur + E_ALO + ((fa + f * 2048) ^ (kh * 64)));
+      if (t + 1 < nk) {
+        stage_b(1, t + 1, (t & 1) ^ 1);
+        wait_vmcnt<8>();
+      } else if (PW) {
+        stage_w2(0);
+        wait_vmcnt<2>();
+      } else {
+        wait_vmcnt<0>();
+      }
+    };
+    auto L1 = [&](int t) {
+      const char* cur = smem + (t & 1) * E_BUF;
+#pragma unroll
+      for (int f = 0; f < 2; ++f)
+#pragma unroll
+        for (int kh = 0; kh < 2; ++kh) ldf(whi[f][kh], cur + E_BHI + ((fb + f * 2048) ^ (kh * 64)));
+      if (t + 1 < nk) {
+        stage_a(1, walk_hi, (t & 1) ^ 1);
+        wait_vmcnt<8>();
+      } else if (PW) {
+        stage_w2(1);
+      } else {
+        wait_vmcnt<0>();
+      }
+    };
+    auto L2 = [&](int t) {
+      const char* cur = smem + (t & 1) * E_BUF;
+#pragma unroll
+      for (int f = 0; f < MF1; ++f)
+#pragma unroll
+        for (int kh = 0; kh < 2; ++kh) ldf(xa[f][kh], cur + E_AHI + ((fa + f * 2048) ^ (kh * 64)));
+      if (t + 2 < nk) stage_a(0, walk_lo, t & 1);
+      if (PW && t + 1 == nk) stage_w2(2);
+    };
+    auto L3 = [&](int t) {
+      if (t + 2 < nk) {
+        stage_b(0, t + 2, t & 1);
+        wait_vmcnt<8>();
+      } else if (PW && t + 1 == nk) {
+        stage_w2(3);
+      } else {
+        wait_vmcnt<0>();
+      }
+    };
+    auto M = [&](int ph) {
+      __builtin_amdgcn_s_setprio(1);
+#pragma unroll
+      for (int kh = 0; kh < 2; ++kh)
+#pragma unroll
+        for (int i = 0; i < ((ph < 2) ? MF0 : MF1); ++i)
+#pragma unroll
+          for (int j = 0; j < 2; ++j) {
+            if (ph == 0) mma(acc[i][j], wlo[j][kh], xa[i][kh]);
+            if (ph == 1) mma(acc[i][2 + j], whi[j][kh], xa[i][kh]);
+            if (ph == 2) mma(acc[MF0 + i][2 + j], whi[j][kh], xa[i][kh]);
+            if (ph == 3) mma(acc[MF0 + i][j], wlo[j][kh], xa[i][kh]);
+          }
+      __builtin_amdgcn_s_setprio(0);
+    };
+
+    if (wr == 0) {
+      for (int t = 0; t < nk; ++t) {
+        L0(t);
+        M(0);
+        __builtin_amdgcn_s_barrier();
+        L1(t);
+        M(1);
+        __builtin_amdgcn_s_barrier();
+        L2(t);
+        M(2);
+        __builtin_amdgcn_s_barrier();
+        L3(t);
+        M(3);
+        __builtin_amdgcn_s_barrier();
+      }
     } else {
-      wait_vmcnt<0>();
-    }
-  };
-  auto L2 = [&](int t) {
-    const char* cur = smem + (t & 1) * E_BUF;
-#pragma unroll
-    for (int f = 0; f < MF1; ++f)
-#pragma unroll
-      for (int kh = 0; kh < 2; ++kh) ldf(xa[f][kh], cur + E_AHI + ((fa + f * 2048) ^ (kh * 64)));
-    if (t + 2 < nk) stage_a(0, walk_lo, t & 1);
-    if (PW && t + 1 == nk) stage_w2(2);
-  };
-  auto L3 = [&](int t) {
-    if (t + 2 < nk) {
-      stage_b(0, t + 2, t & 1);
-      wait_vmcnt<8>();
-    } else if (PW && t + 1 == nk) {
-      stage_w2(3);
+      L0(0);
+      __builtin_amdgcn_s_barrier();
+      for (int t = 0; t < nk; ++t) {
+        M(0);
+        L1(t);
+        __builtin_amdgcn_s_barrier();
+        M(1);
+        L2(t);
+        __builtin_amdgcn_s_barrier();
+        M(2);
+        L3(t);
+        __builtin_amdgcn_s_barrier();
+        M(3);
+        if (t + 1 < nk) {
+          L0(t + 1);
+          __builtin_amdgcn_s_barrier();
+        }
+      }
+    }
+    __syncthreads();
+
+    if constexpr (PW) {
+      const int rg = wave >> 2, cg = wave & 3;
+      float sc2[8], bi2[8];
+      {
+        const int n2 = cg * 32 + (lq & 1) * 16 + (lq >> 1) * 8;
+        const f32x4 s0 = *(const f32x4*)(p.scale2 + n2), s1 = *(const f32x4*)(p.scale2 + n2 + 4);
+        const f32x4 b0 = *(const f32x4*)(p.bias2 + n2), b1 = *(const f32x4*)(p.bias2 + n2 + 4);
+#pragma unroll
+        for (int e = 0; e < 4; ++e) {
+          sc2[e] = s0[e];
+          sc2[4 + e] = s1[e];
+          bi2[e] = b0[e];
+          bi2[4 + e] = b1[e];
+        }
+      }
+      f16x8 ykeep[MT][2];
+      od_mfma_results_ready();
+      e8_epilogue_direct<MT, 4, true, EPI>(p, acc, m0 + wr * WROWS, n0 + wc * 64, l15, lq, ykeep);
+      ConvKP p2 = p;
+      p2.scale = p.scale2;
+      p2.bias = p.bias2;
+      p2.act = p.act2;
+      p2.alpha = p.alpha2;
+      p2.res_mode = OD_RES_NONE;
+      p2.out = (void*)p.out2;
+      p2.out_f32 = 0;
+      p2.Cout = p.Cout2;
+      p2.obs = (long long)p.HoWo * p.Cout2;
+      p2.ops = p.Cout2;
+      char* const ybuf = smem + (w2buf ^ 1) * E_BUF;
+      const char* const wbuf = smem + w2buf * E_BUF;
+      const int fy = (rg * 64 + l15) * 128 + ((lq ^ (l15 & 7)) * 16);
+      const int fw = (cg * 32 + l15) * 128 + ((lq ^ (l15 & 7)) * 16);
+#pragma unroll
+      for (int half = 0; half < 2; ++half) {
+        if (wr == half) {
+#pragma unroll
+          for (int i = 0; i < MT; ++i)
+#pragma unroll
+            for (int pr = 0; pr < 2; ++pr) {
+              const int row = i * 16 + l15;
+              const int chunk = (2 * pr + (lq & 1)) * 2 + (lq >> 1);
+              *(f16x8*)(ybuf + wc * E_REGION + row * 128 + ((chunk ^ (row & 7)) * 16)) = ykeep[i][pr];
+            }
+        }
+        asm volatile("s_waitcnt lgkmcnt(0)" ::: "memory");
+        __builtin_amdgcn_s_barrier();
+        f32x4 acc2[4][2];
+#pragma unroll
+        for (int i = 0; i < 4; ++i)
+#pragma unroll
+          for (int f = 0; f < 2; ++f) acc2[i][f] = f32x4{0.f, 0.f, 0.f, 0.f};
+#pragma unroll
+        for (int ks = 0; ks < 4; ++ks)
+#pragma unroll
+          for (int kh = 0; kh < 2; ++kh) {
+            f16x8 wf[2], yf[4];
+#pragma unroll
+            for (int f = 0; f < 2; ++f) wf[f] = *(const f16x8*)(wbuf + ks * E_REGION + ((fw + f * 2048) ^ (kh * 64)));
+#pragma unroll
+            for (int i = 0; i < 4; ++i) yf[i] = *(const f16x8*)(ybuf + ks * E_REGION + ((fy + i * 2048) ^ (kh * 64)));
+#pragma unroll
+            for (int i = 0; i < 4; ++i)
+#pragma unroll
+              for (int f = 0; f < 2; ++f) acc2[i][f] = __builtin_amdgcn_mfma_f32_16x16x32_f16(wf[f], yf[i], acc2[i][f], 0, 0, 0);
+          }
+        od_mfma_results_ready();
+        e8_epilogue_direct<4, 2, false, EPI2>(p2, acc2, m0 + half * WROWS + rg * 64, cg * 32, l15, lq, nullptr, WROWS - rg * 64, sc2, bi2);
+        if (half == 0) {
+          asm volatile("s_waitcnt lgkmcnt(0)" ::: "memory");
+          __builtin_amdgcn_s_barrier();
+        }
+      }
+    } else if (!SEQ && EPI == OD_EPI_RT && p.splitk > 1) {
+      conv_epilogue<E_BN, 2, 4, MT, 4, 512>(p, smem, acc, m0, n0, tid, wr, wc, l15, lq);
+    } else if (SEQ && pw_pass) {
+      ConvKP p2 = p;
+      p2.scale = p.scale2;
+      p2.bias = p.bias2;
+      p2.act = p.act2;
+      p2.alpha = p.alpha2;
+      p2.res_mode = OD_RES_NONE;
+      p2.out = (void*)p.out2;
+      p2.out_f32 = 0;
+      p2.Cout = p.Cout2;
+      p2.obs = (long long)p.HoWo * p.Cout2;
+      p2.ops = p.Cout2;
+      od_mfma_results_ready();
+      e8_epilogue_direct<MT, 4, false, EPI2>(p2, acc, m0 + wr * WROWS, wc * 64, l15, lq);
     } else {
-      wait_vmcnt<0>();
-    }
-  };
-  auto M = [&](int ph) {
-    __builtin_amdgcn_s_setprio(1);
-#pragma unroll
-    for (int kh = 0; kh < 2; ++kh)
-#pragma unroll
-      for (int i = 0; i < ((ph < 2) ? MF0 : MF1); ++i)
-#pragma unroll
-        for (int j = 0; j < 2; ++j) {
-          if (ph == 0) mma(acc[i][j], wlo[j][kh], xa[i][kh]);
-          if (ph == 1) mma(acc[i][2 + j], whi[j][kh], xa[i][kh]);
-          if (ph == 2) mma(acc[MF0 + i][2 + j], whi[j][kh], xa[i][kh]);
-          if (ph == 3) mma(acc[MF0 + i][j], wlo[j][kh], xa[i][kh]);
-        }
-    __builtin_amdgcn_s_setprio(0);
-  };
-
-  if (wr == 0) {
-    for (int t = 0; t < nk; ++t) {
-      L0(t);
-      M(0);
-      __builtin_amdgcn_s_barrier();
-      L1(t);
-      M(1);
-      __builtin_amdgcn_s_barrier();
-      L2(t);
-      M(2);
-      __builtin_amdgcn_s_barrier();
-      L3(t);
-      M(3);
-      __builtin_amdgcn_s_barrier();
-    }
-  } else {
-    L0(0);
-    __builtin_amdgcn_s_barrier();
-    for (int t = 0; t < nk; ++t) {
-      M(0);
-      L1(t);
-      __builtin_amdgcn_s_barrier();
-      M(1);
-      L2(t);
-      __builtin_amdgcn_s_barrier();
-      M(2);
-      L3(t);
-      __builtin_amdgcn_s_barrier();
-      M(3);
-      if (t + 1 < nk) {
-        L0(t + 1);
-        __builtin_amdgcn_s_barrier();
-      }
-    }
-  }
-  __syncthreads();
-
-  if constexpr (PW) {
-    const int rg = wave >> 2, cg = wave & 3;
-    float sc2[8], bi2[8];
-    {
-      const int n2 = cg * 32 + (lq & 1) * 16 + (lq >> 1) * 8;
-      const f32x4 s0 = *(const f32x4*)(p.scale2 + n2), s1 = *(const f32x4*)(p.scale2 + n2 + 4);
-      const f32x4 b0 = *(const f32x4*)(p.bias2 + n2), b1 = *(const f32x4*)(p.bias2 + n2 + 4);
-#pragma unroll
-      for (int e = 0; e < 4; ++e) {
-        sc2[e] = s0[e];
-        sc2[4 + e] = s1[e];
-        bi2[e] = b0[e];
-        bi2[4 + e] = b1[e];
-      }
-    }
-    f16x8 ykeep[MT][2];
-    od_mfma_results_ready();
-    e8_epilogue_direct<MT, 4, true, EPI>(p, acc, m0 + wr * WROWS, n0 + wc * 64, l15, lq, ykeep);
-    ConvKP p2 = p;
-    p2.scale = p.scale2;
-    p2.bias = p.bias2;
-    p2.act = p.act2;
-    p2.alpha = p.alpha2;
-    p2.res_mode = OD_RES_NONE;
-    p2.out = (void*)p.out2;
-    p2.out_f32 = 0;
-    p2.Cout = p.Cout2;
-    p2.obs = (long long)p.HoWo * p.Cout2;
-    p2.ops = p.Cout2;
-    char* const ybuf = smem + (w2buf ^ 1) * E_BUF;
-    const char* const wbuf = smem + w2buf * E_BUF;
-    const int fy = (rg * 64 + l15) * 128 + ((lq ^ (l15 & 7)) * 16);
-    const int fw = (cg * 32 + l15) * 128 + ((lq ^ (l15 & 7)) * 16);
-#pragma unroll
-    for (int half = 0; half < 2; ++half) {
-      if (wr == half) {
-#pragma unroll
-        for (int i = 0; i < MT; ++i)
-#pragma unroll
-          for (int pr = 0; pr < 2; ++pr) {
-            const int row = i * 16 + l15;
-            const int chunk = (2 * pr + (lq & 1)) * 2 + (lq >> 1);
-            *(f16x8*)(ybuf + wc * E_REGION + row * 128 + ((chunk ^ (row & 7)) * 16)) = ykeep[i][pr];
-          }
-      }
-      asm volatile("s_waitcnt lgkmcnt(0)" ::: "memory");
-      __builtin_amdgcn_s_barrier();
-      f32x4 acc2[4][2];
-#pragma unroll
-      for (int i = 0; i < 4; ++i)
-#pragma unroll
-        for (int f = 0; f < 2; ++f) acc2[i][f] = f32x4{0.f, 0.f, 0.f, 0.f};
-#pragma unroll
-      for (int ks = 0; ks < 4; ++ks)
-#pragma unroll
-        for (int kh = 0; kh < 2; ++kh) {
-          f16x8 wf[2], yf[4];
-#pragma unroll
-          for (int f = 0; f < 2; ++f) wf[f] = *(const f16x8*)(wbuf + ks * E_REGION + ((fw + f * 2048) ^ (kh * 64)));
-#pragma unroll
-          for (int i = 0; i < 4; ++i) yf[i] = *(const f16x8*)(ybuf + ks * E_REGION + ((fy + i * 2048) ^ (kh * 64)));
-#pragma unroll
-          for (int i = 0; i < 4; ++i)
-#pragma unroll
-            for (int f = 0; f < 2; ++f) acc2[i][f] = __builtin_amdgcn_mfma_f32_16x16x32_f16(wf[f], yf[i], acc2[i][f], 0, 0, 0);
-        }
       od_mfma_results_ready();
-      e8_epilogue_direct<4, 2, false, EPI2>(p2, acc2, m0 + half * WROWS + rg * 64, cg * 32, l15, lq, nullptr, WROWS - rg * 64, sc2, bi2);
-      if (half == 0) {
-        asm volatile("s_waitcnt lgkmcnt(0)" ::: "memory");
-        __builtin_amdgcn_s_barrier();
-      }
-    }
-  } else if (EPI == OD_EPI_RT && p.splitk > 1) {
-    conv_epilogue<E_BN, 2, 4, MT, 4, 512>(p, smem, acc, m0, n0, tid, wr, wc, l15, lq);
-  } else {
-    od_mfma_results_ready();
-    e8_epilogue_direct<MT, 4, false, EPI>(p, acc, m0 + wr * WROWS, n0 + wc * 64, l15, lq);
+      e8_epilogue_direct<MT, 4, false, EPI>(p, acc, m0 + wr * WROWS, n0 + wc * 64, l15, lq);
+    }
   }
 }
 
+template <int KS, int MF1, int EPI, int EPI2, bool PW, bool SEG>
+__global__ __launch_bounds__(512, 2) void od_conv_8ph(ConvKP p_in) {
+  e8_body<KS, MF1, EPI, EPI2, PW, SEG, false>(p_in);
 }
+
+template <int KS, int MF1, int EPI, int EPI2>
+__global__ __launch_bounds__(512, 2) void od_conv_8ph_seq(ConvKP p_in) {
+  e8_body<KS, MF1, EPI, EPI2, false, false, true>(p_in);
+}
+
+}
diff --git a/object_detector_amd/csrc/conv_common.h b/object_detector_amd/csrc/conv_common.h
--- a/object_detector_amd/csrc/conv_common.h
+++ b/object_detector_amd/csrc/conv_common.h
@@ -309,12 +309,12 @@
 int od_conv_8ph_num_cfgs();
 long od_conv_8ph_tiles(int idx, int M, int Cout);
 double od_conv_8ph_tile_cost(int idx, int nk);
-bool od_conv_8ph_can_fuse_pointwise(const ConvKP& p);
+int od_conv_8ph_can_fuse_pointwise(const ConvKP& p);
 bool od_conv_8ph_select(int idx, const ConvKP& p, int ksize, ConvKernelInfo* info);
-bool od_conv_8ph_variant_mf4(int ksize, bool pw, int epi, int epi2, const void** fn, const char** name);
-bool od_conv_8ph_variant_mf3(int ksize, bool pw, int epi, int epi2, const void** fn, const char** name);
-bool od_conv_8ph_variant_mf2(int ksize, bool pw, int epi, int epi2, const void** fn, const char** name);
-bool od_conv_8ph_variant_mf1(int ksize, bool pw, int epi, int epi2, const void** fn, const char** name);
+bool od_conv_8ph_variant_mf4(int ksize, int pw, int epi, int epi2, const void** fn, const char** name);
+bool od_conv_8ph_variant_mf3(int ksize, int pw, int epi, int epi2, const void** fn, const char** name);
+bool od_conv_8ph_variant_mf2(int ksize, int pw, int epi, int epi2, const void** fn, const char** name);
+bool od_conv_8ph_variant_mf1(int ksize, int pw, int epi, int epi2, const void** fn, const char** name);
 bool od_tconv_small_supported(const od_conv_desc* d);
 int od_tconv_small_prepare(od_ctx* ctx, const od_conv_desc* d, od_launches* L);
 bool od_conv_rdirect_supported(const od_conv_desc* d);
diff --git a/object_detector_amd/csrc/conv_dispatch.hip b/object_detector_amd/csrc/conv_dispatch.hip
--- a/object_detector_amd/csrc/conv_dispatch.hip
+++ b/object_detector_amd/csrc/conv_dispatch.hip
@@ -163,8 +163,9 @@
   return OD_OK;
 }
 
-int conv_choose_cfg(const od_ctx* ctx, const od_conv_desc* d, const ConvKP& p, bool want_stats, int* cfg_out) {
+int conv_choose_cfg(const od_ctx* ctx, const od_conv_desc* d, const ConvKP& p, bool want_stats, int* cfg_out, bool* seq) {
   int cfg = d->tile_cfg;
+  *seq = d->w2 && cfg >= 0 && od_conv_8ph_can_fuse_pointwise(p) == 2;
   if (cfg < 0)
     cfg = pick_cfg(ctx, p.M, d->Cin, d->Cout, d->ksize, !want_stats && !p.tconv && (long long)p.x_bytes < 0x7F000000LL, cfg == -2);
   const int cfg_e8 = od_conv_igemm_num_cfgs();
@@ -227,7 +228,8 @@
     if (!p.tconv && od_conv_stream3_supported(d)) return od_conv_stream3_prepare(ctx, d, L);
   }
   int cfg;
-  if (int rc = conv_choose_cfg(ctx, d, p, want_stats, &cfg)) return rc;
+  bool seq;
+  if (int rc = conv_choose_cfg(ctx, d, p, want_stats, &cfg, &seq)) return rc;
   const bool use_e8 = cfg >= od_conv_igemm_num_cfgs();
   if (grouped && !(use_e8 && d->Cin % 64 == 0)) {
     od_conv_desc q = *d;
@@ -252,7 +254,8 @@
       return OD_ERR_WORKSPACE;
     }
   }
-  if (d->splitk_workspace && d->splitk != 1 && !p.tconv && !want_stats && !grouped) {
+  const bool seq_whole_k = seq && use_e8 && d->splitk == 0;
+  if (d->splitk_workspace && d->splitk != 1 && !seq_whole_k && !p.tconv && !want_stats && !grouped) {
     const int cus = ctx->num_cu;
     const int tiles = p.mtiles * p.ntiles;
     const int nk = od_ceil_div(p.Ktot, k.BK);
@@ -267,11 +270,15 @@
       p.splitk = od_ceil_div(nk, p.steps_per_split);
     }
   }
-  if (d->w2 && use_e8 && od_conv_8ph_can_fuse_pointwise(p)) p.w2 = (const f16*)d->w2;
+  if (d->w2 && use_e8) {
+    const int form = od_conv_8ph_can_fuse_pointwise(p);
+    if (form == 1 || (form == 2 && seq)) p.w2 = (const f16*)d->w2;
+  }
+  const int wgs = (p.w2 && p.ntiles > 1) ? p.mtiles : p.mtiles * p.ntiles * p.splitk;
   if (int rc = conv_select(cfg, d, p, want_stats, &k)) return rc;
   if (int rc = od_ensure_lds(ctx, k.fn, k.lds)) return rc;
   const size_t launch_lds = (use_e8 && p.splitk <= 1 && k.lds > (size_t)128 * 1024) ? (size_t)128 * 1024 : k.lds;
-  if (int rc = od_add_launch(L, {k.name, od_issue_kp, k.fn, dim3(p.mtiles * p.ntiles * p.splitk), dim3(k.threads), launch_lds}, p))
+  if (int rc = od_add_launch(L, {k.name, od_issue_kp, k.fn, dim3(wgs), dim3(k.threads), launch_lds}, p))
     return rc;
   if (p.splitk > 1)
     if (int rc = od_conv_finish_prepare(p, L)) return rc;
@@ -325,7 +332,8 @@
   ConvKP p;
   ConvKernelInfo k;
   int cfg;
-  if (conv_describe(ctx, d, true, &v, &p) || conv_choose_cfg(ctx, &v, p, true, &cfg) || conv_select(cfg, &v, p, true, &k)) return -1;
+  bool seq;
+  if (conv_describe(ctx, d, true, &v, &p) || conv_choose_cfg(ctx, &v, p, true, &cfg, &seq) || conv_select(cfg, &v, p, true, &k)) return -1;
   conv_tile_kp(&v, k, &p);
   return p.mtiles;
 }
diff --git a/object_detector_amd/net.py b/object_detector_amd/net.py
--- a/object_detector_amd/net.py
+++ b/object_detector_amd/net.py
@@ -284,7 +284,7 @@
         taps = []
         for si, (n, ch) in enumerate(W.STAGES, start=1):
             fused_block = self.fuse_blocks and self.lib.od_bottleneck_supported(h // 2, w // 2, ch)
-            ride = self.fuse_blocks and ch == 256 and not fused_block
+            ride = self.fuse_blocks and ch in (256, 512) and not fused_block
             wide = si in self.stream_stages
             if wide:
                 ride = False
```

New measurement: 22750. No clear change (-0.1%).
